# piljoong-jeong/nerf_meets_mlx

Measured on AMD Instinct MI355X. Metric: train+render rays/sec on Lego 800x800 (synthetic), coarse+fine 64+128, higher is better.
Workload: dtype split16 (fp16x2 render / bf16x2 train MFMA operands ~ 22 / 16 significand bits; fp32 accumulate)

## Files before the change

include/nerf_hip.h:

```cpp
#ifndef NERF_HIP_H
#define NERF_HIP_H

#include <stddef.h>
#include <stdint.h>

#ifdef __cplusplus
extern "C" {
#endif

#define NERF_ABI_VERSION 3

#define NERF_OK 0
#define NERF_E_NULL (-1)
#define NERF_E_SHAPE (-2)
#define NERF_E_UNSUPPORTED (-3)
#define NERF_E_HIP (-4)
#define NERF_E_RCCL (-5)

int nerf_abi_version(void);
const char* nerf_last_error(void);

#define NERF_RAY_STRIDE 11

int nerf_pixel_permutation(int64_t* out_idx, int64_t n, int64_t domain, uint64_t seed, uint64_t offset,
                           void* stream);

int nerf_ray_gen(const int64_t* pixel_idx, int64_t n, int H, int W, const double* K_host, const float* c2w_host,
                 float near, float far, float* rays, int64_t* coords, void* stream);

int nerf_sample_batch(int64_t n, int H, int W, uint64_t seed, uint64_t offset, const double* K_host, const float* c2w_host,
                      float near, float far, const float* image, float* rays, float* target, int64_t* pixel_idx,
                      void* stream);

int nerf_sample_batch_rgba(int64_t n, int H, int W, uint64_t seed, uint64_t offset, const double* K_host, const float* c2w_host,
                           float near, float far, const float* image, float* rays, float* target, int64_t* pixel_idx,
                           void* stream);

int nerf_gather_rows(const float* src, int64_t n_src, const int64_t* idx, int64_t n, int channels, float* out,
                     void* stream);

int nerf_ndc_rays(float* rays, int64_t n, int H, int W, float focal, float near, void* stream);

int nerf_sample_coarse(const float* rays, int64_t B, int n, int lindisp, float perturb, const float* t_rand,
                       float* z, void* stream);

int nerf_add_noise_z(const float* z_in, const float* t_rand, int64_t B, int n, float strength, float* z_out,
                     void* stream);

int nerf_importance_sample(const float* z, const float* weights, const float* u, int64_t B, int n, int N, float eps,
                           float* z_new, float* z_merged, float* cdf, int64_t* inds, void* stream);

int nerf_encode_freq(const float* x, int64_t M, int D, int n_freqs, int freq_mode, float* out, void* stream);

int nerf_encode_sinusoidal(const float* x, int64_t M, int D, int n_freqs, const float* freqs_host,
                           int include_input, float* out, void* stream);

int nerf_sh_encode(const float* dirs, int64_t M, int degree, float* out, void* stream);

int nerf_hashgrid_forward(const float* x, int64_t M, const float* tables, int L, int log2_T, int F,
                          const int* resolutions_host, float* out, void* stream);
int nerf_hashgrid_backward(const float* x, int64_t M, const float* d_out, int L, int log2_T, int F,
                           const int* resolutions_host, float* d_tables, void* stream);

int nerf_ngp_encode(const float* rays, const float* z, int64_t B, int n, const float* tables, int L, int log2_T,
                    int F, const int* resolutions_host, int sh_degree, float pos_scale, float pos_offset, float* x_out,
                    float* pts_out, void* stream);
int nerf_hashgrid_backward_rays(const float* rays, const float* z, int64_t B, int n, const float* d_out, int L,
                                int log2_T, int F, const int* resolutions_host, float pos_scale, float pos_offset,
                                float* d_tables, void* stream);

int nerf_hashgrid_backward_ex(const float* x, int64_t M, const float* d_out, int L, int log2_T, int F,
                              const int* resolutions_host, int level_lo, int level_hi, int fixed_point, void* d_tables,
                              void* stream);
int nerf_hashgrid_backward_rays_ex(const float* rays, const float* z, int64_t B, int n, const float* d_out, int L,
                                   int log2_T, int F, const int* resolutions_host, float pos_scale, float pos_offset,
                                   int level_lo, int level_hi, int fixed_point, void* d_tables, void* stream);

int nerf_hashgrid_forward_lw(const float* x, int64_t M, const float* tables, int L, int log2_T, int F,
                             const int* resolutions_host, const float* level_weights_host, float* out, void* stream);
int nerf_ngp_encode_lw(const float* rays, const float* z, int64_t B, int n, const float* tables, int L, int log2_T,
                       int F, const int* resolutions_host, const float* level_weights_host, int sh_degree,
                       float pos_scale, float pos_offset, float* x_out, float* pts_out, void* stream);
int nerf_hashgrid_backward_ex_lw(const float* x, int64_t M, const float* d_out, int L, int log2_T, int F,
                                 const int* resolutions_host, const float* level_weights_host, int level_lo,
                                 int level_hi, int fixed_point, void* d_tables, void* stream);
int nerf_hashgrid_backward_rays_ex_lw(const float* rays, const float* z, int64_t B, int n, const float* d_out, int L,
                                      int log2_T, int F, const int* resolutions_host, const float* level_weights_host,
                                      float pos_scale, float pos_offset, int level_lo, int level_hi, int fixed_point,
                                      void* d_tables, void* stream);

int nerf_composite_forward(const float* raw, const float* z, const float* rays, int64_t B, int n,
                           float raw_noise_std, const float* noise, int white_bkgd, float* rgb, float* disp,
                           float* acc, float* weights, float* depth, void* stream);

int nerf_composite_backward(const float* raw, const float* z, const float* rays, int64_t B, int n,
                            float raw_noise_std, const float* noise, int white_bkgd, const float* d_rgb,
                            const float* d_acc, const float* d_depth, float* d_raw, void* stream);

int nerf_mse_loss_grad(const float* pred, const float* target, int64_t count, float grad_scale, float* loss_out,
                       float* d_pred, void* stream);

int nerf_composite_mse_backward(const float* raw, const float* z, const float* rays, int64_t B, int n, int white_bkgd,
                                const float* target, float grad_scale, float* loss_out, float* rgb, float* d_raw,
                                void* stream);

int nerf_ssim_sums(const float* pred, const float* gt, int N, int C, int H, int W, const float* window_host,
                   int w_size, float c1, float c2, double* sums, void* stream);

typedef struct nerf_mlp_arch {
  int n_layers;
  int width;
  int in_pos;
  int in_dir;
  int skip_layer;
  int use_viewdirs;
  int out_ch;
  int precision;
} nerf_mlp_arch;

int64_t nerf_mlp_param_count(const nerf_mlp_arch* arch);
int64_t nerf_mlp_packed_bytes(const nerf_mlp_arch* arch);
int nerf_mlp_pack(const nerf_mlp_arch* arch, const float* params, void* packed, void* stream);

int64_t nerf_mlp_acts_bytes(const nerf_mlp_arch* arch, int64_t M);
int64_t nerf_mlp_dz_bytes(const nerf_mlp_arch* arch, int64_t M);

int nerf_mlp_forward(const nerf_mlp_arch* arch, const void* packed, const float* x, int64_t M, float* out,
                     void* stream);
int nerf_mlp_forward_train(const nerf_mlp_arch* arch, const void* packed, const float* x, int64_t M, float* out,
                           void* acts, void* stream);

int nerf_query_fused(const nerf_mlp_arch* arch, const void* packed, const float* rays, const float* z, int64_t B,
                     int n, int freq_mode, float* raw, void* acts, void* stream);

int nerf_mlp_backward(const nerf_mlp_arch* arch, const void* packed, const void* acts, const float* d_raw,
                      int64_t M, void* dz, float* grads, void* stream);
int nerf_mlp_backward_inputs(const nerf_mlp_arch* arch, const void* packed, const void* acts, const float* d_raw,
                             int64_t M, void* dz, float* grads, float* d_x, void* stream);

int nerf_mlp_debug_width(const nerf_mlp_arch* arch, int kind, int layer);
int nerf_mlp_debug_read(const nerf_mlp_arch* arch, const void* store, int kind, int layer, int64_t M, float* out,
                        void* stream);

int nerf_ngp_query_fused(const nerf_mlp_arch* arch, const void* packed, const float* rays, const float* z, int64_t B,
                         int n, const float* tables, int L, int log2_T, int F, const int* resolutions_host,
                         int sh_degree, float pos_scale, float pos_offset, float* raw, void* acts, void* stream);
int nerf_ngp_query_fused_h(const nerf_mlp_arch* arch, const void* packed, const float* rays, const float* z, int64_t B,
                           int n, const float* tables, const void* tables_half, int L, int log2_T, int F,
                           const int* resolutions_host, int sh_degree, float pos_scale, float pos_offset, float* raw,
                           void* acts, void* stream);
int nerf_ngp_query_fused_lw(const nerf_mlp_arch* arch, const void* packed, const float* rays, const float* z, int64_t B,
                            int n, const float* tables, const void* tables_half, int L, int log2_T, int F,
                            const int* resolutions_host, const float* level_weights_host, int sh_degree, float pos_scale,
                            float pos_offset, float* raw, void* acts, void* stream);


int nerf_occ_points(int log2_res, int64_t cell0, int64_t count, uint64_t seed, uint64_t update, float pos_scale,
                    float pos_offset, float* rays_out, float* z_out, void* stream);
int nerf_occ_merge(float* density, const float* raw, int64_t count, float decay, void* stream);
int64_t nerf_occ_finalize_workspace_bytes(int log2_res);
int nerf_occ_finalize(const float* density, int log2_res, float thr_cap, void* workspace, float* thr_out, uint32_t* bits,
                      void* stream);
int64_t nerf_occ_cull_workspace_bytes(int64_t B, int n);
int nerf_occ_cull(const float* rays, const float* z, int64_t B, int n, const uint32_t* bits, int log2_res, float pos_scale,
                  float pos_offset, void* workspace, int64_t* idx_out, int64_t* count_out, float* rays_out, float* z_out,
                  float* raw_fill, void* stream);
int nerf_scatter_rows(const float* src, const int64_t* idx, int64_t n, int channels, float* dst, int64_t n_dst, void* stream);

#define NERF_MARCH_MAX_STEPS 1024
int64_t nerf_occ_march_workspace_bytes(int64_t B);
int nerf_occ_march_count(const float* rays, int64_t B, const float* jitter, float jitter_const, const uint32_t* bits, int log2_res,
                         float pos_scale, float pos_offset, float step_world, int march_steps, void* workspace, int64_t* offsets,
                         void* stream);
int nerf_occ_march_write(const float* rays, int64_t B, const float* jitter, float jitter_const, const uint32_t* bits, int log2_res,
                         float pos_scale, float pos_offset, float step_world, int march_steps, void* workspace, int64_t* offsets,
                         float* rows_out, float* z_out, void* stream);
#define NERF_OCC_RELU 0
#define NERF_OCC_EXP 1
int nerf_occ_merge_ex(float* density, const float* raw, int64_t count, float decay, int activation, void* stream);

int nerf_composite_packed_forward(const float* raw, const float* z, const int64_t* offsets, int64_t B, int64_t K, float step_world,
                                  int white_bkgd, float* rgb, float* acc, float* depth, void* stream);
int nerf_composite_packed_mse_backward(const float* raw, const int64_t* offsets, int64_t B, int64_t K, float step_world,
                                       int white_bkgd, const float* target, float grad_scale, float* loss_out, float* rgb,
                                       float* d_raw, void* stream);

int nerf_composite_packed_distortion(const float* raw, const float* z, const int64_t* offsets, const float* rays, int64_t B,
                                     int64_t K, float step_world, int march_steps, int white_bkgd, float* rgb, float* acc,
                                     float* depth, float* dist, void* stream);
int nerf_composite_packed_mse_dist_backward(const float* raw, const float* z, const int64_t* offsets, const float* rays, int64_t B,
                                            int64_t K, float step_world, int march_steps, int white_bkgd, const float* target,
                                            float grad_scale, float dist_weight, float* loss_out, float* dist_out, float* rgb,
                                            float* d_raw, void* stream);

int nerf_composite_packed_forward_bg(const float* raw, const float* z, const int64_t* offsets, int64_t B, int64_t K, float step_world,
                                     const float* bg, int bg_stride, float* rgb, float* acc, float* depth, void* stream);
int nerf_composite_packed_distortion_bg(const float* raw, const float* z, const int64_t* offsets, const float* rays, int64_t B,
                                        int64_t K, float step_world, int march_steps, const float* bg, int bg_stride, float* rgb,
                                        float* acc, float* depth, float* dist, void* stream);
int nerf_composite_packed_mse_backward_bg(const float* raw, const int64_t* offsets, int64_t B, int64_t K, float step_world,
                                          const float* target_rgba, const float* bg, float grad_scale, float* loss_out, float* rgb,
                                          float* d_raw, void* stream);
int nerf_composite_packed_mse_dist_backward_bg(const float* raw, const float* z, const int64_t* offsets, const float* rays, int64_t B,
                                               int64_t K, float step_world, int march_steps, const float* target_rgba,
                                               const float* bg, float grad_scale, float dist_weight, float* loss_out,
                                               float* dist_out, float* rgb, float* d_raw, void* stream);

#define NERF_ERT_TERMINATED 1
int64_t nerf_ert_march_workspace_bytes(int64_t B);
int nerf_ert_init(int64_t B, int32_t* istate, float* fstate, int32_t* live, void* stream);
int nerf_ert_march_count(const float* rays, int64_t B, const float* jitter, float jitter_const, const uint32_t* bits, int log2_res,
                         float pos_scale, float pos_offset, float step_world, int march_steps, const int32_t* live, int64_t A,
                         const int32_t* istate, int max_new, void* workspace, int64_t* totals, void* stream);
int nerf_ert_march_write(const float* rays, int64_t B, const float* jitter, float jitter_const, const uint32_t* bits, int log2_res,
                         float pos_scale, float pos_offset, float step_world, int march_steps, const int32_t* live, int64_t A,
                         int32_t* istate, int max_new, void* workspace, int64_t* offsets, int32_t* live_out, float* rows_out,
                         float* z_out, void* stream);
int nerf_ert_fold(const float* raw, const float* z, const int64_t* offsets, const int32_t* live, int64_t A, int64_t B, int64_t K,
                  float step_world, float min_transmittance, int32_t* istate, float* fstate, void* stream);
int nerf_ert_finish(const int32_t* istate, const float* fstate, int64_t B, int white_bkgd, float* rgb, float* acc, float* depth,
                    int32_t* samples, void* stream);
int nerf_ert_finish_bg(const int32_t* istate, const float* fstate, int64_t B, const float* bg, int bg_stride, float* rgb, float* acc,
                       float* depth, int32_t* samples, void* stream);

#define NERF_MESH_MAX_RES 512
int64_t nerf_mesh_workspace_bytes(int res);
int nerf_mesh_points(int res, const float* lo_host, const float* hi_host, int64_t p0, int64_t count, float* rays_out, float* z_out,
                     void* stream);
int nerf_mesh_count(const float* vol, int res, float iso, void* workspace, int64_t* totals, void* stream);
int nerf_mesh_write_vertices(const float* vol, int res, float iso, const float* lo_host, const float* hi_host, void* workspace,
                             int64_t V, float* verts, float* normals, float* color_rows, void* stream);
int nerf_mesh_write_faces(const float* vol, int res, float iso, void* workspace, int64_t F, int32_t* faces, void* stream);

int64_t nerf_ccl_workspace_bytes(int res);
int nerf_ccl_label(const float* vol, int res, float iso, void* workspace, int32_t* labels, void* stream);
int nerf_ccl_sizes(const int32_t* labels, int res, int32_t* sizes, int64_t* stats, void* stream);
int nerf_ccl_filter(const float* vol, const int32_t* labels, const int32_t* sizes, const int64_t* stats, int res, float iso,
                    int64_t min_voxels, int largest_only, float* out, void* stream);

#define NERF_MORPH_MAX_RADIUS 16
int64_t nerf_morph_workspace_bytes(int res);
int nerf_morph_erode(const float* vol, int res, float iso, int radius, void* workspace, float* core, int64_t* stats2, void* stream);
int nerf_morph_reconstruct(const float* vol, const float* kept, int res, float iso, int radius, void* workspace, float* out,
                           int64_t* stats2, void* stream);


#define NERF_TSDF_MAX_VIEWS 16
typedef struct nerf_tsdf_view {
  float c2w[12];
  float fx, fy, cx, cy;
} nerf_tsdf_view;
int nerf_tsdf_reset(float* D, float* Wt, uint8_t* flags, int res, void* stream);
int nerf_tsdf_integrate(float* D, float* Wt, uint8_t* flags, int res, const float* lo_host, const float* hi_host,
                        const nerf_tsdf_view* views_host, int n, int H, int W, const float* depth, const float* acc, float trunc,
                        float acc_min, float far, int carve, void* stream);
int nerf_tsdf_volume(const float* D, const float* Wt, const uint8_t* flags, int res, int min_views, float* vol_out, void* stream);

#define NERF_SIMPLIFY_MEAN 0
#define NERF_SIMPLIFY_QUADRIC 1
int64_t nerf_simplify_workspace_bytes(int64_t V, int64_t F, int grid);
int nerf_simplify_cluster(const float* verts, const float* normals, const float* colors, int64_t V, const int32_t* faces, int64_t F,
                          const float* lo_host, const float* hi_host, int grid, void* workspace, int64_t* tri_keys, void* stream);
int nerf_simplify_count(const int64_t* sorted_keys, const int64_t* perm, int64_t V, const int32_t* faces, int64_t F, int grid,
                        void* workspace, int64_t* totals, void* stream);
int nerf_simplify_write(int64_t V, const int32_t* faces, int64_t F, const float* lo_host, const float* hi_host, int grid,
                        int placement, void* workspace, int64_t V_out, int64_t F_out, float* verts_out, float* normals_out,
                        float* colors_out, float* color_rows, int32_t* faces_out, void* stream);

int64_t nerf_smooth_workspace_bytes(int64_t V, int64_t F);
int nerf_smooth_build(int64_t V, const int32_t* faces, int64_t F, void* workspace, void* stream);
int nerf_smooth_run(const float* verts_in, int64_t V, const float* lo_host, const float* hi_host, int iterations, float lambda,
                    float mu, void* workspace, float* verts_out, void* stream);
int nerf_smooth_normals(const float* verts, int64_t V, const float* lo_host, const float* hi_host, void* workspace,
                        float* normals_out, float* color_rows, void* stream);

// ... 93 lines not shown
```

nerf_meets_mlx_amd/_native.py:

```python
import ctypes as C
import os

import torch

_HERE = os.path.dirname(os.path.abspath(__file__))
LIB_PATH = os.environ.get("NERF_HIP_LIB", os.path.join(_HERE, "libnerf_hip.so"))

_P, _I64, _I, _F, _U64 = C.c_void_p, C.c_int64, C.c_int, C.c_float, C.c_uint64
SIGNATURES = {
    "nerf_abi_version": (_I, []),
    "nerf_last_error": (C.c_char_p, []),
    "nerf_pixel_permutation": (_I, [_P, _I64, _I64, _U64, _U64, _P]),
    "nerf_ray_gen": (_I, [_P, _I64, _I, _I, C.POINTER(C.c_double), C.POINTER(C.c_float), _F, _F, _P, _P, _P]),
    "nerf_sample_batch": (_I, [_I64, _I, _I, _U64, _U64, C.POINTER(C.c_double), C.POINTER(C.c_float), _F, _F, _P, _P, _P, _P, _P]),
    "nerf_sample_batch_rgba": (_I, [_I64, _I, _I, _U64, _U64, C.POINTER(C.c_double), C.POINTER(C.c_float), _F, _F, _P, _P, _P, _P, _P]),
    "nerf_gather_rows": (_I, [_P, _I64, _P, _I64, _I, _P, _P]),
    "nerf_ndc_rays": (_I, [_P, _I64, _I, _I, _F, _F, _P]),
    "nerf_sample_coarse": (_I, [_P, _I64, _I, _I, _F, _P, _P, _P]),
    "nerf_add_noise_z": (_I, [_P, _P, _I64, _I, _F, _P, _P]),
    "nerf_importance_sample": (_I, [_P, _P, _P, _I64, _I, _I, _F, _P, _P, _P, _P, _P]),
    "nerf_encode_freq": (_I, [_P, _I64, _I, _I, _I, _P, _P]),
    "nerf_encode_sinusoidal": (_I, [_P, _I64, _I, _I, C.POINTER(C.c_float), _I, _P, _P]),
    "nerf_sh_encode": (_I, [_P, _I64, _I, _P, _P]),
    "nerf_hashgrid_forward": (_I, [_P, _I64, _P, _I, _I, _I, C.POINTER(C.c_int), _P, _P]),
    "nerf_hashgrid_backward": (_I, [_P, _I64, _P, _I, _I, _I, C.POINTER(C.c_int), _P, _P]),
    "nerf_ngp_encode": (_I, [_P, _P, _I64, _I, _P, _I, _I, _I, C.POINTER(C.c_int), _I, C.c_float, C.c_float, _P, _P, _P]),
    "nerf_ngp_query_fused": (_I, [_P, _P, _P, _P, _I64, _I, _P, _I, _I, _I, C.POINTER(C.c_int), _I, C.c_float, C.c_float, _P, _P, _P]),
    "nerf_ngp_query_fused_h": (_I, [_P, _P, _P, _P, _I64, _I, _P, _P, _I, _I, _I, C.POINTER(C.c_int), _I, C.c_float, C.c_float, _P, _P, _P]),
    "nerf_hashgrid_backward_rays": (_I, [_P, _P, _I64, _I, _P, _I, _I, _I, C.POINTER(C.c_int), C.c_float, C.c_float, _P, _P]),
    "nerf_hashgrid_backward_ex": (_I, [_P, _I64, _P, _I, _I, _I, C.POINTER(C.c_int), _I, _I, _I, _P, _P]),
    "nerf_hashgrid_backward_rays_ex": (_I, [_P, _P, _I64, _I, _P, _I, _I, _I, C.POINTER(C.c_int), C.c_float, C.c_float, _I, _I, _I, _P, _P]),
    "nerf_hashgrid_forward_lw": (_I, [_P, _I64, _P, _I, _I, _I, C.POINTER(C.c_int), C.POINTER(C.c_float), _P, _P]),
    "nerf_ngp_encode_lw": (_I, [_P, _P, _I64, _I, _P, _I, _I, _I, C.POINTER(C.c_int), C.POINTER(C.c_float), _I, C.c_float, C.c_float, _P, _P, _P]),
    "nerf_ngp_query_fused_lw": (_I, [_P, _P, _P, _P, _I64, _I, _P, _P, _I, _I, _I, C.POINTER(C.c_int), C.POINTER(C.c_float), _I, C.c_float, C.c_float, _P, _P, _P]),
    "nerf_hashgrid_backward_ex_lw": (_I, [_P, _I64, _P, _I, _I, _I, C.POINTER(C.c_int), C.POINTER(C.c_float), _I, _I, _I, _P, _P]),
    "nerf_hashgrid_backward_rays_ex_lw": (_I, [_P, _P, _I64, _I, _P, _I, _I, _I, C.POINTER(C.c_int), C.POINTER(C.c_float), C.c_float, C.c_float, _I, _I, _I, _P, _P]),
    "nerf_composite_forward": (_I, [_P, _P, _P, _I64, _I, _F, _P, _I, _P, _P, _P, _P, _P, _P]),
    "nerf_composite_backward": (_I, [_P, _P, _P, _I64, _I, _F, _P, _I, _P, _P, _P, _P, _P]),
    "nerf_mse_loss_grad": (_I, [_P, _P, _I64, _F, _P, _P, _P]),
    "nerf_composite_mse_backward": (_I, [_P, _P, _P, _I64, _I, _I, _P, _F, _P, _P, _P, _P]),
    "nerf_ssim_sums": (_I, [_P, _P, _I, _I, _I, _I, C.POINTER(C.c_float), _I, _F, _F, _P, _P]),
    "nerf_mlp_param_count": (_I64, [_P]),
    "nerf_mlp_packed_bytes": (_I64, [_P]),
    "nerf_mlp_pack": (_I, [_P, _P, _P, _P]),
    "nerf_mlp_acts_bytes": (_I64, [_P, _I64]),
    "nerf_mlp_dz_bytes": (_I64, [_P, _I64]),
    "nerf_mlp_forward": (_I, [_P, _P, _P, _I64, _P, _P]),
    "nerf_mlp_forward_train": (_I, [_P, _P, _P, _I64, _P, _P, _P]),
    "nerf_query_fused": (_I, [_P, _P, _P, _P, _I64, _I, _I, _P, _P, _P]),
    "nerf_mlp_backward": (_I, [_P, _P, _P, _P, _I64, _P, _P, _P]),
    "nerf_mlp_backward_inputs": (_I, [_P, _P, _P, _P, _I64, _P, _P, _P, _P]),
    "nerf_mlp_debug_width": (_I, [_P, _I, _I]),
    "nerf_mlp_debug_read": (_I, [_P, _P, _I, _I, _I64, _P, _P]),
    "nerf_render_workspace_bytes": (_I64, [_I64, _I, _I]),
    "nerf_render_rays_fused": (_I, [_P, _P, _P, _P, _I64, _I, _I, _P, _I, _I, _P, _P, _P, _P, _P, _P, _P, _P, _P, _P]),
    "nerf_comm_unique_id": (_I, [C.c_char_p]),
    "nerf_comm_init": (_I, [C.POINTER(C.c_void_p), _I, _I, C.c_char_p]),
    "nerf_allreduce_grads": (_I, [_P, _P, _I64, _P]),
    "nerf_comm_destroy": (_I, [_P]),
    "nerf_set_option": (_I, [C.c_char_p, _I]),
    "nerf_get_option": (_I, [C.c_char_p]),
    "nerf_adam_step": (_I, [_P, _P, _P, _P, _I64, _F, _F, _F, _F, _I, _I, _F, _P]),
    "nerf_adam_step_ex": (_I, [_P, _P, _P, _P, _I64, _F, _F, _F, _F, _I, _I, _F, _I, _I, _P]),
    "nerf_adam_step_shadow": (_I, [_P, _P, _P, _P, _I64, _F, _F, _F, _F, _I, _I, _F, _I, _I, _P, _P]),
    "nerf_occ_points": (_I, [_I, _I64, _I64, _U64, _U64, _F, _F, _P, _P, _P]),
    "nerf_occ_merge": (_I, [_P, _P, _I64, _F, _P]),
    "nerf_occ_finalize_workspace_bytes": (_I64, [_I]),
    "nerf_occ_finalize": (_I, [_P, _I, _F, _P, _P, _P, _P]),
    "nerf_occ_cull_workspace_bytes": (_I64, [_I64, _I]),
    "nerf_occ_cull": (_I, [_P, _P, _I64, _I, _P, _I, _F, _F, _P, _P, _P, _P, _P, _P, _P]),
    "nerf_scatter_rows": (_I, [_P, _P, _I64, _I, _P, _I64, _P]),
    "nerf_occ_merge_ex": (_I, [_P, _P, _I64, _F, _I, _P]),
    "nerf_occ_march_workspace_bytes": (_I64, [_I64]),
    "nerf_occ_march_count": (_I, [_P, _I64, _P, _F, _P, _I, _F, _F, _F, _I, _P, _P, _P]),
    "nerf_occ_march_write": (_I, [_P, _I64, _P, _F, _P, _I, _F, _F, _F, _I, _P, _P, _P, _P, _P]),
    "nerf_composite_packed_forward": (_I, [_P, _P, _P, _I64, _I64, _F, _I, _P, _P, _P, _P]),
    "nerf_composite_packed_mse_backward": (_I, [_P, _P, _I64, _I64, _F, _I, _P, _F, _P, _P, _P, _P]),
    "nerf_composite_packed_distortion": (_I, [_P, _P, _P, _P, _I64, _I64, _F, _I, _I, _P, _P, _P, _P, _P]),
    "nerf_composite_packed_mse_dist_backward": (_I, [_P, _P, _P, _P, _I64, _I64, _F, _I, _I, _P, _F, _F, _P, _P, _P, _P, _P]),
    "nerf_composite_packed_forward_bg": (_I, [_P, _P, _P, _I64, _I64, _F, _P, _I, _P, _P, _P, _P]),
    "nerf_composite_packed_distortion_bg": (_I, [_P, _P, _P, _P, _I64, _I64, _F, _I, _P, _I, _P, _P, _P, _P, _P]),
    "nerf_composite_packed_mse_backward_bg": (_I, [_P, _P, _I64, _I64, _F, _P, _P, _F, _P, _P, _P, _P]),
    "nerf_composite_packed_mse_dist_backward_bg": (_I, [_P, _P, _P, _P, _I64, _I64, _F, _I, _P, _P, _F, _F, _P, _P, _P, _P, _P]),
    "nerf_ert_march_workspace_bytes": (_I64, [_I64]),
    "nerf_ert_init": (_I, [_I64, _P, _P, _P, _P]),
    "nerf_ert_march_count": (_I, [_P, _I64, _P, _F, _P, _I, _F, _F, _F, _I, _P, _I64, _P, _I, _P, _P, _P]),
    "nerf_ert_march_write": (_I, [_P, _I64, _P, _F, _P, _I, _F, _F, _F, _I, _P, _I64, _P, _I, _P, _P, _P, _P, _P, _P]),
    "nerf_ert_fold": (_I, [_P, _P, _P, _P, _I64, _I64, _I64, _F, _F, _P, _P, _P]),
    "nerf_ert_finish": (_I, [_P, _P, _I64, _I, _P, _P, _P, _P, _P]),
    "nerf_ert_finish_bg": (_I, [_P, _P, _I64, _P, _I, _P, _P, _P, _P, _P]),
    "nerf_mesh_workspace_bytes": (_I64, [_I]),
    "nerf_mesh_points": (_I, [_I, C.POINTER(C.c_float), C.POINTER(C.c_float), _I64, _I64, _P, _P, _P]),
    "nerf_mesh_count": (_I, [_P, _I, _F, _P, _P, _P]),
    "nerf_mesh_write_vertices": (_I, [_P, _I, _F, C.POINTER(C.c_float), C.POINTER(C.c_float), _P, _I64, _P, _P, _P, _P]),
    "nerf_mesh_write_faces": (_I, [_P, _I, _F, _P, _I64, _P, _P]),
    "nerf_ccl_workspace_bytes": (_I64, [_I]),
    "nerf_ccl_label": (_I, [_P, _I, _F, _P, _P, _P]),
    "nerf_ccl_sizes": (_I, [_P, _I, _P, _P, _P]),
    "nerf_ccl_filter": (_I, [_P, _P, _P, _P, _I, _F, _I64, _I, _P, _P]),
    "nerf_morph_workspace_bytes": (_I64, [_I]),
    "nerf_morph_erode": (_I, [_P, _I, _F, _I, _P, _P, _P, _P]),
    "nerf_morph_reconstruct": (_I, [_P, _P, _I, _F, _I, _P, _P, _P, _P]),
    "nerf_tsdf_reset": (_I, [_P, _P, _P, _I, _P]),
    "nerf_tsdf_integrate": (_I, [_P, _P, _P, _I, C.POINTER(C.c_float), C.POINTER(C.c_float), C.POINTER(C.c_float), _I, _I, _I, _P, _P,
                                _F, _F, _F, _I, _P]),
    "nerf_tsdf_volume": (_I, [_P, _P, _P, _I, _I, _P, _P]),
    "nerf_simplify_workspace_bytes": (_I64, [_I64, _I64, _I]),
    "nerf_simplify_cluster": (_I, [_P, _P, _P, _I64, _P, _I64, C.POINTER(C.c_float), C.POINTER(C.c_float), _I, _P, _P, _P]),
    "nerf_simplify_count": (_I, [_P, _P, _I64, _P, _I64, _I, _P, _P, _P]),
    "nerf_simplify_write": (_I, [_I64, _P, _I64, C.POINTER(C.c_float), C.POINTER(C.c_float), _I, _I, _P, _I64, _I64, _P, _P, _P, _P,
                                _P, _P]),
    "nerf_smooth_workspace_bytes": (_I64, [_I64, _I64]),
    "nerf_smooth_build": (_I, [_I64, _P, _I64, _P, _P]),
    "nerf_smooth_run": (_I, [_P, _I64, C.POINTER(C.c_float), C.POINTER(C.c_float), _I, _F, _F, _P, _P, _P]),
    "nerf_smooth_normals": (_I, [_P, _I64, C.POINTER(C.c_float), C.POINTER(C.c_float), _P, _P, _P, _P]),
    "nerf_texture_layout": (_I, [_I64, _I, C.POINTER(C.c_int64)]),
    "nerf_texture_rows": (_I, [_P, _P, _I64, _P, _I64, _I, _I64, _I64, _P, _P]),
    "nerf_texture_store": (_I, [_P, _I64, _P, _I64, _I, _I64, _I64, _P, _P]),
    "nerf_texture_uv": (_I, [_I64, _I, _P, _P]),
    "nerf_texture_sample": (_I, [_P, _P, _P, _I64, _P, _I64, _I, _P, _P, _I64, _P, _P, _P]),
    "nerf_raster_clear": (_I, [_P, _I, _I, _P, _P]),
    "nerf_raster_draw": (_I, [_P, _I64, _P, _I64, _I64, C.POINTER(C.c_float), _I, _I, _F, _I, _I, _P, _P, _P]),
    "nerf_raster_resolve": (_I, [_P, _P, _I64, _P, _I64, C.POINTER(C.c_float), _I, _I, _F, _P, _P, _P, _P, _P]),
    "nerf_raster_shade": (_I, [_P, _P, _P, _I64, _I64, _P, _P, _P, _I, _I, _I, _P, _P]),
    "nerf_project_accumulate": (_I, [_P, _P, _I64, _P, _I64, _I, _I64, _I64, C.POINTER(C.c_float), _I, _I, _I, _P, _P, _P, _F, _F, _F, _F,
                                    _I, _P, _P]),
    "nerf_project_finish": (_I, [_P, _I64, _I, _I64, _I64, _I, _P, _P, _P, _P]),
    "nerf_mip_levels": (_I, [_I, C.POINTER(C.c_int32)]),
    "nerf_mip_reduce": (_I, [_P, _I64, _I, _P, _I64, _I64, _P]),
    "nerf_mip_lod": (_I, [_P, _I64, _P, _I64, C.POINTER(C.c_float), _F, _I, _F, _P, _P]),
    "nerf_mip_sample": (_I, [C.POINTER(C.c_void_p), _I64, _I, _P, _P, _P, _I, _I64, _P, _P]),
    "nerf_surface_cdf_workspace_bytes": (_I64, [_I64]),
    "nerf_surface_cdf": (_I, [_P, _I64, _P, _I64, C.POINTER(C.c_float), C.POINTER(C.c_float), _P, _P, _P]),
    "nerf_surface_sample": (_I, [_P, _I64, _P, _I64, _P, _I64, _I64, _U64, _P, _P, _P]),
    "nerf_meshdist_workspace_bytes": (_I64, [_I64, _I]),
    "nerf_meshdist_count": (_I, [_P, _I64, _P, _I64, C.POINTER(C.c_float), C.POINTER(C.c_float), _I, _P, _P, _P]),
    "nerf_meshdist_build": (_I, [_P, _I64, _P, _I64, C.POINTER(C.c_float), C.POINTER(C.c_float), _I, _P, _P, _I64, _P]),
    "nerf_meshdist_query": (_I, [_P, _I64, _P, _I64, _P, _I64, C.POINTER(C.c_float), C.POINTER(C.c_float), _I, _P, _P, _I64, _P, _P,
                                _P]),
    "nerf_bvh_workspace_bytes": (_I64, [_I64]),
    "nerf_bvh_keys": (_I, [_P, _I64, _P, _I64, C.POINTER(C.c_float), C.POINTER(C.c_float), _P, _P]),
    "nerf_bvh_build": (_I, [_P, _I64, _P, _I64, _P, _P, _P]),
    "nerf_bvh_query": (_I, [_P, _I64, _P, _I64, _P, _I64, C.POINTER(C.c_float), C.POINTER(C.c_float), _P, _P, _P, _P]),
    "nerf_closest_points": (_I, [_P, _I64, _P, _I64, _P, _I64, _P, _P, _P]),
}


class MlpArch(C.Structure):
    _fields_ = [("n_layers", _I), ("width", _I), ("in_pos", _I), ("in_dir", _I), ("skip_layer", _I),
                ("use_viewdirs", _I), ("out_ch", _I), ("precision", _I)]


class NerfHipError(RuntimeError):
    pass


_lib = None


def lib():
    global _lib
    if _lib is None:
        if not os.path.exists(LIB_PATH):
            raise NerfHipError(
                f"{LIB_PATH} not found: build it with `python -c 'import __graft_entry__ as g; g.build()'` "
                "(hipcc --offload-arch=gfx950).  There is no CPU fallback.")
        L = C.CDLL(LIB_PATH)
        for name, (res, args) in SIGNATURES.items():
            fn = getattr(L, name)
            fn.restype, fn.argtypes = res, args
        _lib = L
    return _lib


def check(rc: int):
    if rc != 0:
        msg = lib().nerf_last_error().decode(errors="replace")
        if rc in (-1, -2, -3):
            raise ValueError(f"libnerf_hip error {rc}: {msg}")
        raise NerfHipError(f"libnerf_hip error {rc}: {msg}")


def ptr(t):
    if t is None:
        return None
    if not t.is_cuda:
        raise ValueError("libnerf_hip kernels need tensors on the ROCm device (there is no CPU path)")
    if not t.is_contiguous():
        raise ValueError("libnerf_hip kernels need contiguous tensors")
    return C.c_void_p(t.data_ptr())


def stream():
    return C.c_void_p(torch.cuda.current_stream().cuda_stream)


def f32(t, device=None):
    if not torch.is_tensor(t):
        t = torch.as_tensor(t)
    if device is not None:
        t = t.to(device)
    return t.to(torch.float32).contiguous()
```

nerf_meets_mlx_amd/csrc/mlp.hip:

```cpp
#include "common.h"
#include "mlp_ring.h"
#include "mlp_layout.h"
#include "mlp_frag.h"
#include "mlp_arch2.h"
#include "mlp_input2.h"
#include "mlp_pack.h"
#include "hash_common.h"
#include "mlp_params.h"
#include "mlp_model.h"
#include "dw_split.h"
#include <limits.h>
#include <string.h>


namespace nerf {

extern int g_hash_combine_max_res;








template <int ST, int KS, int NT, bool RELU, bool MASKOUT, class WS, class SINK = NoSink>
__device__ __forceinline__ void layer_fwd(WS& ws, int fbase, int bias_slot, const bf16x8 (&in)[ST][KS],
                                          bf16x8 (&out)[ST][2 * NT], u32x4 (&mask)[ST], int lane,
                                          const SINK& sink = SINK()) {
  const int h = lane >> 5;
  f32x16 prev[ST];
#pragma unroll
  for (int nt = 0; nt < NT; ++nt) {
    f32x16 acc[ST];
    acc_init_bias(acc[0], ws, bias_slot + 32 * nt, h);
#pragma unroll
    for (int t = 1; t < ST; ++t) acc[t] = acc[0];
#pragma unroll
    for (int ks = 0; ks < KS; ++ks) {
      const bf16x8 a = next_frag(ws, fbase + nt * KS + ks, lane);
#pragma unroll
      for (int t = 0; t < ST; ++t) acc[t] = __builtin_amdgcn_mfma_f32_32x32x16_bf16(a, in[t][ks], acc[t], 0, 0, 0);
      if (nt > 0) {
#pragma unroll
        for (int q = 0; q < 4; ++q)
          if (quarter_pos(KS, q) == ks) {
#pragma unroll
            for (int t = 0; t < ST; ++t) {
              finish_quarter<RELU, MASKOUT>(prev[t], q, nt - 1, out[t][2 * nt - 2], out[t][2 * nt - 1], mask[t]);
              if (q == 3) { sink.put(t, 2 * nt - 2, out[t][2 * nt - 2]); sink.put(t, 2 * nt - 1, out[t][2 * nt - 1]); }
            }
          }
      }
    }
#pragma unroll
    for (int t = 0; t < ST; ++t) prev[t] = acc[t];
  }
#pragma unroll
  for (int q = 0; q < 4; ++q)
#pragma unroll
    for (int t = 0; t < ST; ++t)
      finish_quarter<RELU, MASKOUT>(prev[t], q, NT - 1, out[t][2 * NT - 2], out[t][2 * NT - 1], mask[t]);
#pragma unroll
  for (int t = 0; t < ST; ++t) { sink.put(t, 2 * NT - 2, out[t][2 * NT - 2]); sink.put(t, 2 * NT - 1, out[t][2 * NT - 1]); }
}


template <int ST, int MODE, bool STORE, class WS>
__device__ __forceinline__ void fwd_tiles(const FwdArgs& a, WS& ws, int64_t tile0, int64_t ntiles, int lane, PassQueue* pq = nullptr) {
  const int r = lane & 31, h = lane >> 5;
  bf16x8 pe[ST][4], dpe[ST][2];
  if (pq) pq->ask(ws_wave(ws), lane);
#pragma unroll
  for (int t = 0; t < ST; ++t) {
    int64_t tile = tile0 + t; if (tile >= ntiles) tile = ntiles - 1;
    const int64_t m = clamp_sample(tile * 32 + r, a.M);
    if (MODE == 0) {
      const float* row = a.x + m * 90;
#pragma unroll
      for (int ks = 0; ks < 4; ++ks) row_pairs<CvtBf16>(row, ks, h, 63, pe[t][ks]);
#pragma unroll
      for (int ks = 0; ks < 2; ++ks) row_pairs<CvtBf16>(row + 63, ks, h, 27, dpe[t][ks]);
    } else {
      const Sample sm = load_sample(a.rays, a.z, m, a.n);
#if NERF_ABLATE == 3
      for (int q = 0; q < 4; ++q) for (int j = 0; j < 8; ++j) pe[t][q][j] = (__bf16)sm.p[j % 3];
      for (int q = 0; q < 2; ++q) for (int j = 0; j < 8; ++j) dpe[t][q][j] = (__bf16)sm.d[j % 3];
      if (false)
#endif
      {
      encode_pairs<SinRevFract, CvtBf16, 0, 63, 10>(sm.p, a.fr.pos, h, pe[t][0]); encode_pairs<SinRevFract, CvtBf16, 1, 63, 10>(sm.p, a.fr.pos, h, pe[t][1]);
      encode_pairs<SinRevFract, CvtBf16, 2, 63, 10>(sm.p, a.fr.pos, h, pe[t][2]); encode_pairs<SinRevFract, CvtBf16, 3, 63, 10>(sm.p, a.fr.pos, h, pe[t][3]);
      encode_pairs<SinRevFract, CvtBf16, 0, 27, 4>(sm.d, a.fr.dir, h, dpe[t][0]); encode_pairs<SinRevFract, CvtBf16, 1, 27, 4>(sm.d, a.fr.dir, h, dpe[t][1]);
      }
    }
  }
  if (pq) pq->publish(ws_wave(ws));
  int bad[ST];
#pragma unroll
  for (int t = 0; t < ST; ++t)
  {
    bad[t] = nonfinite_flags<32>(nonfinite_bits(pe[t][0]) | nonfinite_bits(pe[t][1]) | nonfinite_bits(pe[t][2]) | nonfinite_bits(pe[t][3]),
                                 nonfinite_bits(dpe[t][0]) | nonfinite_bits(dpe[t][1]));
    asm volatile("" : "+v"(bad[t]));
  }
#define store(slot0, t, frags, count) \
  do { if (STORE) { store_frags<count>(a.acts, tile0 + (t), a.astride, slot0, frags, r, h); ws.note_stores(count); } } while (0)
#pragma unroll
  for (int t = 0; t < ST; ++t) { store(L::A_PE, t, pe[t], 4); store(L::A_DPE, t, dpe[t], 2); }

  bf16x8 ha[ST][16], hb[ST][16];
  u32x4 mk[ST];
#define SINK(slot0) FragSink<STORE>{a.acts, tile0, a.astride, slot0, r, h}
#define MASK_BEGIN() do { _Pragma("unroll") for (int t = 0; t < ST; ++t) mk[t] = u32x4{0u, 0u, 0u, 0u}; } while (0)
#define MASK_STORE(layer) do { if (STORE) { _Pragma("unroll") for (int t = 0; t < ST; ++t) \
    *reinterpret_cast<u32x4*>(frag_ptr(a.acts, tile0 + t, a.astride, L::A_MASK + (layer), r, h)) = mk[t]; ws.note_stores(ST); } } while (0)
  MASK_BEGIN();
  layer_fwd<ST, 4, 8, true, STORE>(ws, L::F_L0, 0, pe, ha, mk, lane, SINK(L::A_H0));
  MASK_STORE(0);
  MASK_BEGIN();
  layer_fwd<ST, 16, 8, true, STORE>(ws, L::F_L1 + 0 * 128, 256, ha, hb, mk, lane, SINK(L::A_H0 + 16));
  MASK_STORE(1);
  MASK_BEGIN();
  layer_fwd<ST, 16, 8, true, STORE>(ws, L::F_L1 + 1 * 128, 512, hb, ha, mk, lane, SINK(L::A_H0 + 32));
  MASK_STORE(2);
  MASK_BEGIN();
  layer_fwd<ST, 16, 8, true, STORE>(ws, L::F_L1 + 2 * 128, 768, ha, hb, mk, lane, SINK(L::A_H0 + 48));
  MASK_STORE(3);
  MASK_BEGIN();
  layer_fwd<ST, 16, 8, true, STORE>(ws, L::F_L1 + 3 * 128, 1024, hb, ha, mk, lane, SINK(L::A_H0 + 64));
  MASK_STORE(4);
  {
    bf16x8 cat[ST][20];
#pragma unroll
    for (int t = 0; t < ST; ++t) {
      if (STORE && is_ring<WS>::value) {
#pragma unroll
        for (int k = 0; k < 4; ++k) pe[t][k] = *frag_ptr(a.acts, tile0 + t, a.astride, L::A_PE + k, r, h);
      }
#pragma unroll
      for (int k = 0; k < 4; ++k) cat[t][k] = pe[t][k];
#pragma unroll
      for (int k = 0; k < 16; ++k) cat[t][4 + k] = ha[t][k];
    }
    MASK_BEGIN();
    layer_fwd<ST, 20, 8, true, STORE>(ws, L::F_L5, 1280, cat, hb, mk, lane, SINK(L::A_H0 + 80));
    MASK_STORE(5);
  }
  MASK_BEGIN();
  layer_fwd<ST, 16, 8, true, STORE>(ws, L::F_L6, 1536, hb, ha, mk, lane, SINK(L::A_H0 + 96));
  MASK_STORE(6);
  MASK_BEGIN();
  layer_fwd<ST, 16, 8, true, STORE>(ws, L::F_L7, 1792, ha, hb, mk, lane, SINK(L::A_H0 + 112));
  MASK_STORE(7);
  layer_fwd<ST, 16, 8, false, false>(ws, L::F_FA, L::BI_FEAT, hb, ha, mk, lane, SINK(L::A_FEAT));
  float alpha[ST];
  {
    f32x16 acc[ST];
    acc_init_bias(acc[0], ws, L::BI_ALPHA, h);
#pragma unroll
    for (int t = 1; t < ST; ++t) acc[t] = acc[0];
#pragma unroll
    for (int ks = 0; ks < 16; ++ks) {
      const bf16x8 wa = next_frag(ws, L::F_FA + 128 + ks, lane);
#pragma unroll
      for (int t = 0; t < ST; ++t) acc[t] = __builtin_amdgcn_mfma_f32_32x32x16_bf16(wa, hb[t][ks], acc[t], 0, 0, 0);
    }
#pragma unroll
    for (int t = 0; t < ST; ++t) alpha[t] = acc[t][0];
  }
// ... 786 lines not shown
  }
  ws.drain();
}



struct LdsW {
  __device__ __forceinline__ bf16x8 frag(int f, int lane) { return *reinterpret_cast<const bf16x8*>(ring_smem + f * 1024 + lane * 16); }
  __device__ __forceinline__ void note_stores(int) {}
  __device__ __forceinline__ float4 bias4(int slot) { return *reinterpret_cast<const float4*>(ring_smem + 32 * 1024 + slot * 4); }
};
__device__ __forceinline__ void lds_load_stream(const bf16x8* __restrict__ w, const float* __restrict__ bias) {
  for (int i = threadIdx.x; i < 32 * 64; i += blockDim.x) *reinterpret_cast<bf16x8*>(ring_smem + i * 16) = w[i];
  if (bias)
    for (int i = threadIdx.x; i < LN::BI_TOTAL; i += blockDim.x) *reinterpret_cast<float*>(ring_smem + 32 * 1024 + 4 * i) = bias[i];
  __syncthreads();
}


template <bool STORE, bool FUSED, bool LW = false>
__global__ void __launch_bounds__(512) mlp_small_fwd_kernel(SmallArgs a) {
  constexpr int ST = 1;
  lds_load_stream(a.wf, a.bias);
  const int lane0 = threadIdx.x & 63, wv = threadIdx.x >> 6;
  const bool rmaj = FUSED && !STORE && a.ray_major;
  const int64_t ntiles = rmaj ? ((a.B + 31) >> 5) * a.n : (a.M + 31) >> 5;
  LdsW ws;
  for (int64_t tile0 = (int64_t)blockIdx.x * 8 + wv; tile0 < ntiles; tile0 += (int64_t)gridDim.x * 8) {
    int lane = lane0;
    asm volatile("" : "+v"(lane));
    const int r = lane & 31, h = lane >> 5;
    const TileSample ts = small_tile_sample(a, tile0, r, rmaj);
    const int64_t m = ts.m;
    const bool valid = ts.valid;
    bf16x8 in[3];
    if (FUSED) {
      if (a.tables_h) ngp_row<true, LW, CvtBf16>(a, m, h, in);
      else ngp_row<false, LW, CvtBf16>(a, m, h, in);
    } else {
      small_row<CvtBf16>(a.x + m * LN::CIN, h, in);
    }
    bf16x8 xin[ST][2], din[ST][1];
    xin[0][0] = in[0]; xin[0][1] = in[1]; din[0][0] = in[2];
    int bad = nonfinite_flags<32>(nonfinite_bits(xin[0][0]) | nonfinite_bits(xin[0][1]), nonfinite_bits(din[0][0]));
    asm volatile("" : "+v"(bad));
#define SINK(slot0) FragSink<STORE>{a.acts, tile0, a.astride, slot0, r, h}
#define MASK_STORE(layer) do { if (STORE) *reinterpret_cast<u32x4*>(frag_ptr(a.acts, tile0, a.astride, LN::A_MASK + (layer), r, h)) = mk[0]; } while (0)
    if (STORE) { store_frags<2>(a.acts, tile0, a.astride, LN::A_X, xin[0], r, h); store_frags<1>(a.acts, tile0, a.astride, LN::A_DX, din[0], r, h); }
    u32x4 mk[ST];
    bf16x8 h0[ST][4], h1[ST][4], ft[ST][4];
    mk[0] = u32x4{0u, 0u, 0u, 0u};
    layer_fwd<ST, 2, 2, true, STORE>(ws, LN::F_L0, LN::BI_L0, xin, h0, mk, lane, SINK(LN::A_H0));
    MASK_STORE(0);
    mk[0] = u32x4{0u, 0u, 0u, 0u};
    layer_fwd<ST, 4, 2, true, STORE>(ws, LN::F_L1, LN::BI_L1, h0, h1, mk, lane, SINK(LN::A_H1));
    MASK_STORE(1);
    layer_fwd<ST, 4, 2, false, false>(ws, LN::F_FA, LN::BI_FEAT, h1, ft, mk, lane, SINK(LN::A_FEAT));
    float alpha;
    {
      f32x16 acc;
      acc_init_bias(acc, ws, LN::BI_ALPHA, h);
#pragma unroll
      for (int ks = 0; ks < 4; ++ks) acc = __builtin_amdgcn_mfma_f32_32x32x16_bf16(ws.frag(LN::F_FA + 8 + ks, lane), h1[0][ks], acc, 0, 0, 0);
      alpha = acc[0];
    }
    bf16x8 hd[ST][2];
    {
      bf16x8 cat[ST][5];
#pragma unroll
      for (int k = 0; k < 4; ++k) cat[0][k] = ft[0][k];
      cat[0][4] = din[0][0];
      mk[0] = u32x4{0u, 0u, 0u, 0u};
      layer_fwd<ST, 5, 1, true, STORE>(ws, LN::F_DIR, LN::BI_DIR, cat, hd, mk, lane, SINK(LN::A_HD));
      MASK_STORE(2);
    }
    {
      f32x16 acc;
      acc_init_bias(acc, ws, LN::BI_RGB, h);
#pragma unroll
      for (int ks = 0; ks < 2; ++ks) acc = __builtin_amdgcn_mfma_f32_32x32x16_bf16(ws.frag(LN::F_RGB + ks, lane), hd[0][ks], acc, 0, 0, 0);
      if (h == 0 && valid) {
        float4 o; o.x = acc[0]; o.y = acc[1]; o.z = acc[2]; o.w = alpha;
        *reinterpret_cast<float4*>(a.out + m * 4) = poison_raw(o, bad);
      }
    }
#undef SINK
#undef MASK_STORE
  }
}

__global__ void __launch_bounds__(512) mlp_small_bwd_kernel(SmallArgs a) {
  constexpr int ST = 1;
  lds_load_stream(a.wb, nullptr);
  const int lane0 = threadIdx.x & 63, wv = threadIdx.x >> 6;
  const int64_t ntiles = (a.M + 31) >> 5;
  LdsW ws;
  for (int64_t tile0 = (int64_t)blockIdx.x * 8 + wv; tile0 < ntiles; tile0 += (int64_t)gridDim.x * 8) {
    int lane = lane0;
    asm volatile("" : "+v"(lane));
    const int r = lane & 31, h = lane >> 5;
    const int64_t m = tile0 * 32 + r;
    float4 g = make_float4(0.f, 0.f, 0.f, 0.f);
    if (m < a.M && h == 0) g = *reinterpret_cast<const float4*>(a.d_raw + m * 4);
    bf16x8 zrgb[ST][1], zal[ST][1];
#pragma unroll
    for (int j = 0; j < 8; ++j) { zrgb[0][0][j] = (__bf16)0.0f; zal[0][0][j] = (__bf16)0.0f; }
    zrgb[0][0][0] = (__bf16)g.x; zrgb[0][0][1] = (__bf16)g.y; zrgb[0][0][2] = (__bf16)g.z;
    zal[0][0][0] = (__bf16)g.w;
    u32x4 mk[3][ST];
#pragma unroll
    for (int l = 0; l < 3; ++l)
      mk[l][0] = *reinterpret_cast<const u32x4*>(frag_ptr(const_cast<void*>(a.acts), tile0, a.astride, LN::A_MASK + l, r, h));
    store_frags<1>(a.dz, tile0, a.zstride, LN::Z_RGB, zrgb[0], r, h);
    store_frags<1>(a.dz, tile0, a.zstride, LN::Z_A, zal[0], r, h);
#define ZSINK(slot0) FragSink<true>{a.dz, tile0, a.zstride, slot0, r, h}
    bf16x8 zd[ST][2], zf[ST][4], z1[ST][4], z0[ST][4];
    layer_bwd<ST, 1, 1, true>(ws, LN::B_RGB, zrgb, zd, mk[2], lane, ZSINK(LN::Z_D));
    layer_bwd<ST, 2, 2, false>(ws, LN::B_DIR, zd, zf, mk[2], lane, ZSINK(LN::Z_F));
    {
      bf16x8 cat[ST][5];
#pragma unroll
      for (int k = 0; k < 4; ++k) cat[0][k] = zf[0][k];
      cat[0][4] = zal[0][0];
      layer_bwd<ST, 5, 2, true>(ws, LN::B_FA, cat, z1, mk[1], lane, ZSINK(LN::Z_L1));
    }
    layer_bwd<ST, 4, 2, true>(ws, LN::B_L1, z1, z0, mk[0], lane, ZSINK(LN::Z_L0));
#undef ZSINK
    if (a.d_x) {
      f32x16 acc;
#pragma unroll
      for (int i = 0; i < 16; ++i) acc[i] = 0.0f;
#pragma unroll
      for (int ns = 0; ns < 4; ++ns) acc = __builtin_amdgcn_mfma_f32_32x32x16_bf16(ws.frag(LN::B_L0 + ns, lane), z0[0][ns], acc, 0, 0, 0);
      if (m < a.M) {
#pragma unroll
        for (int q = 0; q < 4; ++q) {
          float4 o; o.x = acc[4 * q]; o.y = acc[4 * q + 1]; o.z = acc[4 * q + 2]; o.w = acc[4 * q + 3];
          *reinterpret_cast<float4*>(a.d_x + m * LN::CPOS + 8 * q + 4 * h) = o;
        }
      }
    }
  }
}

static int g_dw_wgs = 0;
static int g_dw_bias = -1;
static int g_bwd_stage = 0;
static int g_dw_ring_cap = 8;
static int g_dw_private = 4;
static int g_dw16_variant = 1;
static int g_dw_narrow_first = 1;
static int g_dw_factor = 1;
static int g_train_fold = 0;
static int g_dw_job_mask = 0;
static int g_mlp_variant = 0;
static int g_ring_wgs = 0;
static int g_ngp_ray_major = 1;
int g_pass_queue = 1;
static int g_ring_split = 1;

static int cu_count() {
  constexpr int MAX_DEVICES = 64;
  static int n[MAX_DEVICES] = {};
  int dev = 0;
  if (hipGetDevice(&dev) != hipSuccess || dev < 0 || dev >= MAX_DEVICES) dev = 0;
  if (n[dev] == 0) {
    int v = 0;
    n[dev] = (hipDeviceGetAttribute(&v, hipDeviceAttributeMultiprocessorCount, dev) == hipSuccess && v > 0) ? v : 256;
  }
  return n[dev];
}
static inline bool dw_factored(const Model& m) { return g_dw_factor && m.can_factor() && !g_dw_job_mask && s16::g_dw_variant != 0; }
static inline bool train_folded(const Model& m) { return g_train_fold && dw_factored(m); }
static inline int ring_wgs() { return g_ring_wgs > 0 ? g_ring_wgs : cu_count(); }
static inline unsigned ring_grid(int64_t ntiles) { return persistent_grid((ntiles + 7) / 8, ring_wgs()); }

struct Option { const char* key; int* var; bool (*rule)(int& v); const char* refusal; };
static bool opt_any(int&) { return true; }
static bool opt_flag(int& v) { v = v ? 1 : 0; return true; }
template <int LO, int HI> static bool opt_clamp(int& v) { v = v < LO ? LO : v > HI ? HI : v; return true; }
static const Option OPTIONS[] = {
    {"mlp_variant", &g_mlp_variant, opt_any, nullptr},
    {"ring_split", &g_ring_split, [](int& v) { return v == 1 || v == 2; }, "nerf_set_option: ring_split must be 1 or 2"},
    {"ring_workgroups", &g_ring_wgs, opt_clamp<0, INT_MAX>, nullptr},
    {"tile_pad16", &g_tile_pad16, opt_clamp<0, INT_MAX>, nullptr},
    {"dw_workgroups", &g_dw_wgs, opt_clamp<0, INT_MAX>, nullptr},
    {"dw_unit_bias", &g_dw_bias, opt_clamp<-1, INT_MAX>, nullptr},
    {"bwd_stage", &g_bwd_stage, opt_any, nullptr},
    {"dw_job_mask", &g_dw_job_mask, opt_any, nullptr},
    {"hash_combine_max_res", &g_hash_combine_max_res, opt_clamp<0, INT_MAX>, nullptr},
    {"ngp_ray_major", &g_ngp_ray_major, opt_flag, nullptr},
    {"dw22_variant", &s16::g_dw_variant, opt_flag, nullptr},
    {"dw16_variant", &g_dw16_variant, opt_clamp<0, 3>, nullptr},
    {"dw_private_tiles", &g_dw_private, opt_clamp<0, 4>, nullptr},
    {"dw_ring_cap", &g_dw_ring_cap, opt_clamp<2, 16>, nullptr},
    {"pass_queue", &g_pass_queue, opt_flag, nullptr},
    {"dw_narrow_first", &g_dw_narrow_first, opt_flag, nullptr},
    {"dw_factor", &g_dw_factor, opt_flag, nullptr},
    {"train_fold", &g_train_fold, opt_flag, nullptr},
    {"f22_tiles", &f22::g_tiles, [](int& v) { return v == 0 || v == 2 || v == 3; }, "nerf_set_option: f22_tiles must be 0 (automatic), 2 or 3"},
};

}

using namespace nerf;

extern "C" int nerf_set_option(const char* key, int value) {
  NERF_REQUIRE(key, NERF_E_NULL, "nerf_set_option: key is NULL");
  NERF_REQUIRE(strcmp(key, "mlp_precision") != 0, NERF_E_UNSUPPORTED,
               "nerf_set_option: \"mlp_precision\" is gone (ABI 3): set nerf_mlp_arch.precision of the model instead");
  for (const Option& o : OPTIONS) {
    if (strcmp(key, o.key)) continue;
    if (!o.rule(value)) return fail(NERF_E_UNSUPPORTED, "%s", o.refusal);
    *o.var = value;
    return NERF_OK;
  }
  return fail(NERF_E_UNSUPPORTED, "nerf_set_option: unknown key '%s'", key);
}

extern "C" int nerf_get_option(const char* key) {
  if (!key) return NERF_OPTION_UNKNOWN;
  for (const Option& o : OPTIONS)
    if (!strcmp(key, o.key)) return *o.var;
  return NERF_OPTION_UNKNOWN;
}

extern "C" int64_t nerf_mlp_param_count(const nerf_mlp_arch* arch) { return resolve(arch).params; }
extern "C" int64_t nerf_mlp_packed_bytes(const nerf_mlp_arch* arch) { return resolve(arch).packed_bytes; }
extern "C" int64_t nerf_mlp_acts_bytes(const nerf_mlp_arch* arch, int64_t M) { return resolve(arch).acts_bytes(M); }
extern "C" int64_t nerf_mlp_dz_bytes(const nerf_mlp_arch* arch, int64_t M) { return resolve(arch).dz_bytes(M); }

#define NERF_ARCH_MSG ": HIP kernels exist for (8x256, skip 4) with in=63+27 view head, or in=40 / no view head / out_ch<=4, and for (2x64, no skip) with in=32+16 view head"
#define NERF_RESOLVE(who)        \
  const Model m = resolve(arch); \
  NERF_REQUIRE(m.ok, NERF_E_UNSUPPORTED, who NERF_ARCH_MSG)

extern "C" int nerf_mlp_pack(const nerf_mlp_arch* arch, const float* params, void* packed, void* stream) {
  NERF_RESOLVE("nerf_mlp_pack");
  NERF_REQUIRE(params && packed, NERF_E_NULL, "nerf_mlp_pack: params/packed is NULL");
  auto s = as_stream(stream);
  bf16x8* wf = m.stream<bf16x8>(packed, S_FWD);
  bf16x8* wb = m.stream<bf16x8>(packed, S_BWD);
  float* bias = m.stream<float>(packed, S_BIAS);
  int rc;
  if (m.shape == Shape::Small) {
    rc = launch<pack_streams_kernel<SmallPack, CvtBf16, true>>("nerf_mlp_pack (2x64 model)", dim3(pack_blocks<SmallPack, true>()), dim3(256), 0, s,
                                                               params, wf, wb, bias, 0);
    if (!rc && m.split()) rc = s16x::small_pack(params, m.stream<void>(packed, S_S16), s);
  } else if (m.shape == Shape::Image) {
    rc = launch<pack_streams_kernel<ImgPack, CvtBf16, true>>("nerf_mlp_pack (image model)", dim3(pack_blocks<ImgPack, true>()), dim3(256), 0, s,
                                                             params, wf, wb, bias, m.out_ch);
    if (!rc && m.split()) rc = s16x::img_pack(params, m.out_ch, m.stream<void>(packed, S_S16), s);
    if (!rc && m.prec == Prec::F32) rc = f32::pack(params, m.stream<void>(packed, S_F32), m.out_ch, s);
  } else {
    rc = launch<pack_kernel>("nerf_mlp_pack", dim3(PACK_BLOCKS + PACK16_BLOCKS), dim3(256), 0, s, params, wf, wb, bias,
                             m.stream<bf16x8>(packed, S_FWD16));
    if (!rc && m.prec == Prec::F32) rc = f32::pack(params, m.stream<void>(packed, S_F32), 0, s);
    if (!rc && m.split()) rc = f22::pack(params, m.stream<void>(packed, S_F22), s);
    if (!rc && m.split()) rc = s16::pack(params, m.stream<void>(packed, S_S16), train_folded(m), s);
  }
  return rc;
}

template <int MODE>
static int launch_fwd(const Model& m, const void* packed, const float* x, const float* rays, const float* z, int64_t M, int n,
                      int freq_mode, float* out, void* acts, void* stream) {
  FwdArgs a;
  a.queue = nullptr;
  a.wf = m.stream<bf16x8>(packed, S_FWD);
  a.bias = m.stream<float>(packed, S_BIAS);
  a.x = x; a.rays = rays; a.z = z; a.M = M; a.n = n; a.out = out; a.acts = acts; a.astride = m.astride();
  fill_freqs(a.fr.pos, a.fr.dir, freq_mode);
  const int64_t ntiles = (M + 31) / 32;
  auto s = as_stream(stream);
  const int variant = (g_mlp_variant == 0) ? (MODE == 1 ? (acts ? 3 : 4) : 1) : g_mlp_variant;
  if ((variant == 4 || variant == 5) && MODE == 1 && !acts) {
    const dim3 g(persistent_grid((M + 255) / 256, ring_wgs()));
    FwdArgs a16 = a;
    a16.queue = passq_slot();
    a16.wf = m.stream<bf16x8>(packed, S_FWD16);
    const char* what = "mlp forward (ring, 16x16x32)";
    if (variant == 4) return launch<mlp_fwd_ring16_kernel<8, 2>, mlp_fwd_ring16_kernel<4, 4>>(what, g, dim3(512), RING16_LDS_BYTES, s, a16);
    return launch<mlp_fwd_ring16_kernel<4, 4>, mlp_fwd_ring16_kernel<8, 2>>(what, g, dim3(256), RING16_LDS_BYTES, s, a16);
  }
  if (variant >= 3 && MODE == 1) {
    a.queue = passq_slot();
    if (acts && g_ring_split == 2) {
      return launch<mlp_fwd_ring_kernel<1, true, SPLIT_NW, SPLIT_CHUNK>>(
          "mlp forward (ring, 2 workgroups per CU)", dim3(persistent_grid((ntiles + SPLIT_NW - 1) / SPLIT_NW, 2 * (int64_t)ring_wgs())),
          dim3(64 * SPLIT_NW), SPLIT_LDS_BYTES, s, a);
    }
    return with_bool(acts != nullptr, [&](auto store) {
      constexpr bool ST = decltype(store)::value;
      return launch<mlp_fwd_ring_kernel<1, ST>, mlp_fwd_ring_kernel<1, !ST>>("mlp forward (ring)", dim3(ring_grid(ntiles)), dim3(512),
                                                                              RING_LDS_BYTES, s, a);
    });
  }
  const int st = variant == 2 ? 2 : 1;
  const int64_t blocks = (ntiles + 4 * st - 1) / (4 * st);
  NERF_REQUIRE(blocks < (1ll << 31), NERF_E_SHAPE, "mlp forward: M too large");
  return with_bool(st == 1, [&](auto one) { return with_bool(acts != nullptr, [&](auto store) {
    return launch<mlp_fwd_kernel<decltype(one)::value ? 1 : 2, MODE, decltype(store)::value>>("mlp forward", dim3((unsigned)blocks), dim3(256),
                                                                                                0, s, a);
  }); });
}


static int view_forward(const Model& m, const void* packed, const float* x, const float* rays, const float* z, int64_t M, int n,
                        int freq_mode, float* out, void* acts, void* stream);

extern "C" int nerf_mlp_forward_train(const nerf_mlp_arch* arch, const void* packed, const float* x, int64_t M,
                                      float* out, void* acts, void* stream) {
  NERF_RESOLVE("nerf_mlp_forward");
  if (M <= 0) return NERF_OK;
  NERF_REQUIRE(packed && x && out, NERF_E_NULL, "nerf_mlp_forward: NULL pointer");
  auto s = as_stream(stream);
  if (m.shape == Shape::Small) {
    SmallArgs a;
    small_args(a, m, packed);
    a.x = x; a.out = out; a.acts = acts; a.M = M;
    if (m.split()) return s16x::small_forward(a, false, dim3(small_grid(small_tiles(a))), s);
    return with_bool(acts != nullptr, [&](auto store) {
      return launch<mlp_small_fwd_kernel<decltype(store)::value, false>>("mlp forward (2x64 model)", dim3(small_grid((M + 31) / 32)), dim3(512),
                                                                         LN::LDS_BYTES, s, a);
    });
  }
  if (m.shape == Shape::Image) {
    if (m.prec == Prec::F32)
      return f32::forward(m.stream<void>(packed, S_F32), x, nullptr, nullptr, M, 1, 0, out, acts, m.out_ch, s);
    ImgArgs a;
    img_args(a, m, packed);
    a.x = x; a.out = out; a.acts = acts; a.M = M;
    if (m.split()) return s16x::img_forward(a, ring_wgs(), s);
    return with_bool(acts != nullptr, [&](auto store) {
      constexpr bool ST = decltype(store)::value;
      return launch<mlp_img_fwd_ring_kernel<ST>, mlp_img_fwd_ring_kernel<!ST>>("mlp forward (image model)", dim3(ring_grid((M + 31) / 32)),
                                                                               dim3(512), RING_LDS_BYTES, s, a);
    });
  }
  return view_forward(m, packed, x, nullptr, nullptr, M, 1, 0, out, acts, stream);
}

static int view_forward(const Model& m, const void* packed, const float* x, const float* rays, const float* z, int64_t M, int n,
                        int freq_mode, float* out, void* acts, void* stream) {
  auto s = as_stream(stream);
  if (m.split() && !acts)
    return f22::forward(m.stream<void>(packed, S_F22), x, rays, z, M, n, freq_mode, out, ring_wgs(), s);
  if (m.split())
    return s16::forward(m.stream<void>(packed, S_S16), m.stream<float>(packed, S_BIAS), x, rays, z, M, n, freq_mode, out, acts,
                        m.astride(), ring_wgs(), train_folded(m), s);
  if (m.prec == Prec::F32) return f32::forward(m.stream<void>(packed, S_F32), x, rays, z, M, n, freq_mode, out, acts, 0, s);
  return x ? launch_fwd<0>(m, packed, x, rays, z, M, n, freq_mode, out, acts, stream)
           : launch_fwd<1>(m, packed, x, rays, z, M, n, freq_mode, out, acts, stream);
}

extern "C" int nerf_mlp_forward(const nerf_mlp_arch* arch, const void* packed, const float* x, int64_t M, float* out,
                                void* stream) {
  return nerf_mlp_forward_train(arch, packed, x, M, out, nullptr, stream);
}

extern "C" int nerf_query_fused(const nerf_mlp_arch* arch, const void* packed, const float* rays, const float* z,
                                int64_t B, int n, int freq_mode, float* raw, void* acts, void* stream) {
  const Model m = resolve(arch);
  NERF_REQUIRE(m.ok && m.shape == Shape::View, NERF_E_UNSUPPORTED, "nerf_query_fused" NERF_ARCH_MSG);
  NERF_REQUIRE(n >= 1, NERF_E_SHAPE, "nerf_query_fused: n must be >= 1");
  if (B <= 0) return NERF_OK;
  NERF_REQUIRE(packed && rays && z && raw, NERF_E_NULL, "nerf_query_fused: NULL pointer");
  NERF_REQUIRE(freq_mode == 0 || freq_mode == 1, NERF_E_UNSUPPORTED, "nerf_query_fused: freq_mode must be 0 or 1");
  NERF_REQUIRE(B * (int64_t)n < (1ll << 31), NERF_E_SHAPE, "nerf_query_fused: B*n must be < 2^31 samples per call");
  return view_forward(m, packed, nullptr, rays, z, B * n, n, freq_mode, raw, acts, stream);
}

static int launch_dw_part(const Model& m, DwArgs& d, int nj, int64_t ntiles, const void* acts, void* dz, float* grads,
                          hipStream_t s, int kind, int slot_base, int max_wgs, int aux_slot = -1) {
  static_assert(DW_SPLIT_MAX_JOBS == DW_MAX_JOBS, "dw_split.h sizes its arrays for DwArgs::jobs");
  DwCost cost[DW_MAX_JOBS];
  constexpr int SHARED_JOB_EXTRA_UNITS = 12;
  for (int j = 0; j < nj; ++j) cost[j] = DwCost{d.jobs[j].nf, d.jobs[j].kf + (d.jobs[j].aux_row0 > 0 ? SHARED_JOB_EXTRA_UNITS : 0)};
  int target_wgs = g_dw_wgs > 0 ? g_dw_wgs : cu_count();
  if (target_wgs > max_wgs) target_wgs = max_wgs;
  const int nw = dw_split(cost, nj, g_dw_bias >= 0 ? g_dw_bias : m.split() ? 2 : 128, target_wgs, (ntiles + 3) / 4, d.splits);
  NERF_REQUIRE(slot_base + nw <= DW_MAX_WGS, NERF_E_SHAPE, "nerf_mlp_backward: dw_workgroups must be <= %d", DW_MAX_WGS);
  bool all_tiny = true;
  for (int j = 0; j < nj; ++j) all_tiny = all_tiny && ((d.jobs[j].nf + 1) / 2) * ((d.jobs[j].kf + 1) / 2) <= 4;
  d.ntiles = (int)ntiles; d.astride = m.astride(); d.zstride = m.zstride();
  d.acts = acts; d.dz = dz; d.grads = grads;
  d.a_lo = m.info->a_lo; d.z_lo = m.info->z_lo; d.ring_cap = g_dw_ring_cap; d.private_max_tiles = g_dw_private;
  d.partial = m.dw_partial(dz, ntiles) + (size_t)slot_base * DW_SLOT_FLOATS;
  d.aux = aux_slot >= 0 ? m.dw_partial(dz, ntiles) + (size_t)aux_slot * DW_SLOT_FLOATS : nullptr;
  int rc;
  if (kind >= 2) {
    rc = launch_dw_wide_kernel(d, nw, kind == 2, s);
  } else if (kind == 1) {
    rc = s16::launch_dw_kernel(d, nw, true, s);
  } else if (g_dw16_variant == 3 || (g_dw16_variant == 1 && all_tiny)) {
    rc = s16::launch_dw_kernel(d, nw, false, s);
  } else {
    rc = launch<mlp_dw_kernel>("mlp dW", dim3(nw), dim3(64 * DW_WAVES), DW_LDS_BYTES, s, d);
  }
  if (rc) return rc;
  return launch<mlp_dw_reduce_kernel>("mlp dW reduce", dim3(257, nj), dim3(256), 0, s, d);
}

static int launch_dw(const Model& m, const void* packed, DwArgs& d, int nj, int64_t ntiles, const void* acts, void* dz, float* grads,
                     hipStream_t s, bool factored) {
  if (g_dw_job_mask) {
    hipError_t e = hipMemsetAsync(grads, 0, sizeof(float) * m.params, s);
    if (e != hipSuccess) return fail(NERF_E_HIP, "nerf_mlp_backward: memset: %s", hipGetErrorString(e));
  }
  const bool split_bf16 = m.split();
  if ((split_bf16 ? s16::g_dw_variant : g_dw16_variant) == 0)
    return launch_dw_part(m, d, nj, ntiles, acts, dz, grads, s, split_bf16 ? 1 : 0, 0, DW_MAX_WGS);
// ... 210 lines not shown
```

nerf_meets_mlx_amd/csrc/mlp22.h:

```cpp
#pragma once
#ifdef __HIPCC__
#include <hip/hip_runtime.h>
#endif
#include <stdint.h>
#include "mlp_index.h"

#ifndef NERF_F22_FOLD
#define NERF_F22_FOLD 1
#endif

namespace nerf {
namespace f22 {

constexpr int P_L0 = 0, P_L1 = 32, P_L5 = 544, P_L6 = 704, P_L7 = 832, P_HEADS = 960;
#if NERF_F22_FOLD
constexpr int P_ALPHA = P_HEADS, P_DIR = P_ALPHA + 8, P_RGB = P_DIR + 72, F_PAIRS = P_RGB + 4;
#else
constexpr int P_FEAT = P_HEADS, P_ALPHA = P_FEAT + 128, P_DIR = P_ALPHA + 8, P_RGB = P_DIR + 72, F_PAIRS = P_RGB + 4;
#endif
constexpr int F_CHUNK = 32;
constexpr int F_FRAGS = 2 * F_PAIRS, F_STREAM = (F_FRAGS + F_CHUNK - 1) / F_CHUNK * F_CHUNK, CHUNKS = F_STREAM / F_CHUNK;
constexpr int F_PADDED = 2368, BIAS_FLOATS = 2496;
constexpr int64_t PACKED_BYTES = (int64_t)F_PADDED * 1024 + (int64_t)BIAS_FLOATS * 4;
static_assert(F_STREAM <= F_PADDED && F_FRAGS % 4 == 0, "f22 stream layout");

#if NERF_F22_FOLD
constexpr int SRC_ZERO = -1, SRC_FOLD = -2;
struct Src { int p, n, k; };
__host__ __device__ constexpr Src src_param(int p) { return Src{p, 0, 0}; }
__host__ __device__ constexpr Src src_pos_chan(int row_base, int ks, int g, int j) {
  return pos_chan16(ks, g, j) >= 0 ? src_param(row_base + pos_chan16(ks, g, j)) : Src{SRC_ZERO, 0, 0};
}
__host__ __device__ constexpr Src stream_src(int fp, int i, int g, int j) {
  if (fp < P_L1) return src_pos_chan(L::P_W0 + (16 * (fp / 2) + i) * 63, fp % 2, g, j);
  if (fp < P_L5 || (fp >= P_L6 && fp < P_HEADS)) {
    const int q = fp < P_L5 ? fp - P_L1 : fp - P_L6, l = (fp < P_L5 ? 1 : 6) + q / 128, r = q % 128;
    return src_param(L::pw(l) + (16 * (r / 8) + i) * 256 + kperm16(r % 8, g, j));
  }
  if (fp < P_L6) {
    const int q = fp - P_L5, n = 16 * (q / 10) + i, ks = q % 10;
    return ks < 2 ? src_pos_chan(L::P_W5 + n * 319, ks, g, j) : src_param(L::P_W5 + n * 319 + 63 + kperm16(ks - 2, g, j));
  }
  if (fp < P_DIR) return i == 0 ? src_param(L::P_WA + kperm16(fp - P_ALPHA, g, j)) : Src{SRC_ZERO, 0, 0};
  if (fp < P_RGB) {
    const int q = fp - P_DIR, n = 16 * (q / 9) + i, ks = q % 9;
    if (ks < 8) return Src{SRC_FOLD, n, kperm16(ks, g, j)};
    return dir_chan16(g, j) >= 0 ? src_param(L::P_WD + n * 283 + 256 + dir_chan16(g, j)) : Src{SRC_ZERO, 0, 0};
  }
  if (fp < F_PAIRS) return i < 3 ? src_param(L::P_WR + i * 128 + kperm16(fp - P_RGB, g, j)) : Src{SRC_ZERO, 0, 0};
  return Src{SRC_ZERO, 0, 0};
}
#endif

#ifdef __HIPCC__
extern int g_tiles;
int pack(const float* params, void* packed22, hipStream_t s);
int forward(const void* packed22, const float* x, const float* rays, const float* z, int64_t M, int n, int freq_mode,
            float* out, int persistent_wgs, hipStream_t s);
#endif

}
}
```

nerf_meets_mlx_amd/csrc/mlp22.hip:

```cpp
#include "mlp_layout.h"
#include "mlp22.h"

#ifndef NERF_F22_PIN
#define NERF_F22_PIN 1
#endif
#ifndef NERF_F22_AGPR
#define NERF_F22_AGPR 1
#endif
#ifndef NERF_F22_MIXSUB
#define NERF_F22_MIXSUB 1
#endif
#ifndef NERF_F22_RG3
#define NERF_F22_RG3 4
#endif
#ifndef NERF_F22_PARK
#define NERF_F22_PARK (NERF_F22_FOLD ? 2 : 1)
#endif
#ifndef NERF_F22_IGLP
#define NERF_F22_IGLP 0
#endif

namespace nerf {
namespace f22 {

typedef _Float16 h8 __attribute__((ext_vector_type(8)));
typedef _Float16 h2 __attribute__((ext_vector_type(2)));
typedef float f32x2 __attribute__((ext_vector_type(2)));
typedef unsigned int u32x4 __attribute__((ext_vector_type(4)));

constexpr float LO_SCALE = 2048.0f, LO_INV = 1.0f / 2048.0f;
constexpr float F16_MIN_NORMAL = 6.103515625e-05f;
static_assert(F_CHUNK == RING_CHUNK && CHUNKS == (F_FRAGS + RING_CHUNK - 1) / RING_CHUNK && CHUNKS * RING_CHUNK <= F_PADDED, "f22 ring chunks");
static_assert(P_L0 == L16::F_L0 && P_L1 == L16::F_L1 && P_L5 == L16::F_L5 && P_L6 == L16::F_L6 && P_L7 == L16::F_L7 && P_HEADS == L16::F_FA, "f22 trunk");
#if NERF_F22_FOLD
static_assert(F_PAIRS == L::F16_TOTAL - 128 && CHUNKS == 66 && F_FRAGS % RING_CHUNK == (2 * L::F16_TOTAL) % RING_CHUNK, "f22 folded stream");
#else
static_assert(F_PAIRS == L::F16_TOTAL && P_ALPHA == L16::F_FA + 128 && P_DIR == L16::F_DIR && P_RGB == L16::F_RGB && CHUNKS == 74, "f22 stream layout");
#endif

struct HiLo { unsigned hi, lo; };
__device__ __forceinline__ HiLo split2(float v0, float v1) {
  const f32x2 v = {v0, v1};
  const h2 hh = __builtin_convertvector(v, h2);
#if NERF_F22_MIXSUB
  const f32x2 r = {__builtin_fmaf((float)hh[0], -LO_SCALE, v0 * LO_SCALE), __builtin_fmaf((float)hh[1], -LO_SCALE, v1 * LO_SCALE)};
#else
  const f32x2 r = {(v0 - (float)hh[0]) * LO_SCALE, (v1 - (float)hh[1]) * LO_SCALE};
#endif
  return HiLo{__builtin_bit_cast(unsigned, hh), __builtin_bit_cast(unsigned, __builtin_convertvector(r, h2))};
}

constexpr int PACK_THREADS = (F_PADDED / 2) * 64 + BIAS_FLOATS;
__global__ void __launch_bounds__(256) pack22_kernel(const float* __restrict__ p, u32x4* __restrict__ wf,
                                                     float* __restrict__ bias) {
  const int t = blockIdx.x * 256 + threadIdx.x;
  if (t < (F_PADDED / 2) * 64) {
    const int fp = t >> 6, lane = t & 63;
    u32x4 hi = {0u, 0u, 0u, 0u}, lo = {0u, 0u, 0u, 0u};
    if (fp < F_PAIRS) {
#if NERF_F22_FOLD
      float fold[8] = {0.0f, 0.0f, 0.0f, 0.0f, 0.0f, 0.0f, 0.0f, 0.0f};
      if (fp >= P_DIR && fp < P_RGB && (fp - P_DIR) % 9 < 8) {
        const float* __restrict__ wd = p + L::P_WD + (16 * ((fp - P_DIR) / 9) + (lane & 15)) * 283;
        const float* __restrict__ wfk = p + L::P_WF + kperm16((fp - P_DIR) % 9, lane >> 4, 0);
        double acc[8] = {0.0, 0.0, 0.0, 0.0, 0.0, 0.0, 0.0, 0.0};
#pragma unroll 4
        for (int f = 0; f < 256; ++f) {
          const double a = (double)wd[f];
#pragma unroll
          for (int e = 0; e < 8; ++e) acc[e] = __builtin_fma(a, (double)wfk[f * 256 + 16 * (e >> 2) + (e & 3)], acc[e]);
        }
#pragma unroll
        for (int e = 0; e < 8; ++e) fold[e] = (float)acc[e];
      }
#endif
#pragma unroll
      for (int j = 0; j < 8; j += 2) {
        float w[2];
        _Float16 wh[2], wl[2];
#pragma unroll
        for (int e = 0; e < 2; ++e) {
#if NERF_F22_FOLD
          const Src src = stream_src(fp, lane & 15, lane >> 4, j + e);
          w[e] = src.p >= 0 ? p[src.p] : src.p == SRC_FOLD ? fold[j + e] : 0.0f;
#else
          w[e] = fwd_src16(p, fp, lane & 15, lane >> 4, j + e);
#endif
          wh[e] = __builtin_fabsf(w[e]) < F16_MIN_NORMAL ? (_Float16)0.0f : (_Float16)w[e];
          wl[e] = (_Float16)((w[e] - (float)wh[e]) * LO_SCALE);
        }
        const h2 a = {wh[0], wh[1]}, b = {wl[0], wl[1]};
        hi[j >> 1] = __builtin_bit_cast(unsigned, a);
        lo[j >> 1] = __builtin_bit_cast(unsigned, b);
      }
    }
    wf[(2 * fp) * 64 + lane] = hi;
    wf[(2 * fp + 1) * 64 + lane] = lo;
  } else if (t < PACK_THREADS) {
    const int s = t - (F_PADDED / 2) * 64;
    float v = 0.0f;
    if (s < 2048) v = p[L::pb(s >> 8) + (s & 255)];
#if NERF_F22_FOLD
    else if (s < L::BI_ALPHA) v = 0.0f;
    else if (s < L::BI_DIR) v = (s == L::BI_ALPHA) ? p[L::P_BA] : 0.0f;
    else if (s < L::BI_RGB) {
      const float* __restrict__ wd = p + L::P_WD + (s - L::BI_DIR) * 283;
      double acc = 0.0;
      for (int f = 0; f < 256; ++f) acc = __builtin_fma((double)wd[f], (double)p[L::P_BF + f], acc);
      v = (float)(acc + (double)p[L::P_BD + (s - L::BI_DIR)]);
    }
#else
    else if (s < L::BI_ALPHA) v = p[L::P_BF + (s - L::BI_FEAT)];
    else if (s < L::BI_DIR) v = (s == L::BI_ALPHA) ? p[L::P_BA] : 0.0f;
    else if (s < L::BI_RGB) v = p[L::P_BD + (s - L::BI_DIR)];
#endif
    else v = (s - L::BI_RGB) < 3 ? p[L::P_BR + (s - L::BI_RGB)] : 0.0f;
    bias[s] = v;
  }
}

template <int COUNT>
__device__ __forceinline__ void split_slots(const float (&v)[COUNT], u32x4* hi, u32x4* lo) {
#pragma unroll
  for (int j = 0; j < COUNT; j += 2) {
    const HiLo q = split2(v[j], v[j + 1]);
    hi[j >> 3][(j & 7) >> 1] = q.hi; lo[j >> 3][(j & 7) >> 1] = q.lo;
  }
}
struct SplitF16 {
  static __device__ __forceinline__ void pack(const float (&v)[8], u32x4& hi, u32x4& lo) { split_slots<8>(v, &hi, &lo); }
};

__device__ __forceinline__ f32x4 mfma16(const u32x4& a, const u32x4& b, const f32x4& c) {
#if NERF_ABLATE == 41 || NERF_ABLATE == 42
  return c;
#endif
  return __builtin_amdgcn_mfma_f32_16x16x32_f16(__builtin_bit_cast(h8, a), __builtin_bit_cast(h8, b), c, 0, 0, 0);
}

template <int NS, int KS, int NT, bool RELU, class WS, int PARK_LDS = 0>
__device__ __forceinline__ void layer22(WS& ws, int pbase, int bias_slot, const u32x4 (&ih)[NS][KS], const u32x4 (&il)[NS][KS],
                                        u32x4 (&oh)[NS][NT / 2], u32x4 (&ol)[NS][NT / 2], int lane, unsigned park_addr = 0u, unsigned park2_addr = 0u) {
  const int g = lane >> 4;
  f32x4 pm[NS], pc[NS];
  if (PARK_LDS) asm volatile("ds_write_b128 %0, %1" :: "v"(park_addr), "v"(il[NS - 1][KS - 1]) : "memory");
  if (PARK_LDS >= 2)
    asm volatile("ds_write_b32 %0, %1\n\tds_write_b32 %0, %2 offset:1024\n\tds_write_b32 %0, %3 offset:2048\n\tds_write_b32 %0, %4 offset:6144"
                 :: "v"(park2_addr), "v"(il[NS - 2][KS - 1][0]), "v"(il[NS - 2][KS - 1][1]), "v"(il[NS - 2][KS - 1][2]), "v"(il[NS - 2][KS - 1][3]) : "memory");
#if NERF_F22_IGLP >= 0
  __builtin_amdgcn_iglp_opt(NERF_F22_IGLP);
#endif
  constexpr int NP = 2 * NS;
  auto piece = [&](int nt, int pcs, f32x4 (&m)[NS], f32x4 (&c)[NS]) {
    const int s = pcs >> 1, i = 2 * (pcs & 1);
#if NERF_ABLATE == 41 || NERF_ABLATE == 42
    return;
#endif
#if NERF_F22_PIN
    if (pcs == 0) {
#pragma unroll
      for (int t = 0; t < NS; ++t) asm volatile("" : "+v"(m[t]), "+v"(c[t]));
    }
#endif
    float v0 = __builtin_fmaf(c[s][i], LO_INV, m[s][i]), v1 = __builtin_fmaf(c[s][i + 1], LO_INV, m[s][i + 1]);
    if (RELU) { v0 = __builtin_elementwise_maximum(v0, 0.0f); v1 = __builtin_elementwise_maximum(v1, 0.0f); }
    const HiLo q = split2(v0, v1);
    oh[s][nt >> 1][2 * (nt & 1) + (i >> 1)] = q.hi; ol[s][nt >> 1][2 * (nt & 1) + (i >> 1)] = q.lo;
#if NERF_F22_AGPR
    if ((nt & 1) && i == 2) asm volatile("" : "+a"(oh[s][nt >> 1]), "+a"(ol[s][nt >> 1]));
#endif
  };
  auto piece_at = [](int q) { return NS == 2 ? (KS >= 8 ? 1 + 2 * q : (q * KS) / 4) : (KS >= 8 ? 1 + (q * (KS - 1)) / NP : (q * KS) / NP); };
#pragma unroll
  for (int nt = 0; nt < NT; ++nt) {
    const float4 b = ws.bias4(bias_slot + 16 * nt + 4 * g);
    f32x4 m[NS], c[NS];
    m[0][0] = b.x; m[0][1] = b.y; m[0][2] = b.z; m[0][3] = b.w;
    c[0] = f32x4{0.0f, 0.0f, 0.0f, 0.0f};
#pragma unroll
    for (int t = 1; t < NS; ++t) { m[t] = m[0]; c[t] = c[0]; }
#pragma unroll
    for (int ks = 0; ks < KS; ++ks) {
      const int fp = pbase + nt * KS + ks;
      const u32x4 ah = __builtin_bit_cast(u32x4, next_frag(ws, 2 * fp, lane));
      const u32x4 al = __builtin_bit_cast(u32x4, next_frag(ws, 2 * fp + 1, lane));
      if (NS == 2) {
        m[0] = mfma16(ah, ih[0][ks], m[0]);
        c[0] = mfma16(ah, il[0][ks], c[0]);
        m[1] = mfma16(ah, ih[1][ks], m[1]);
        c[1] = mfma16(ah, il[1][ks], c[1]);
        c[0] = mfma16(al, ih[0][ks], c[0]);
        c[1] = mfma16(al, ih[1][ks], c[1]);
      } else {
#pragma unroll
        for (int t = 0; t < NS; ++t) {
          m[t] = mfma16(ah, ih[t][ks], m[t]);
          if (PARK_LDS && t == NS - 1 && ks == KS - 1) {
            u32x4 b;
            asm volatile("ds_read_b128 %0, %1\n\ts_waitcnt lgkmcnt(0)" : "=v"(b) : "v"(park_addr) : "memory");
            c[t] = mfma16(ah, b, c[t]);
          } else if (PARK_LDS >= 2 && t == NS - 2 && ks == KS - 1) {
            u32x4 b;
            asm volatile("ds_read_b32 %0, %4\n\tds_read_b32 %1, %4 offset:1024\n\tds_read_b32 %2, %4 offset:2048\n\tds_read_b32 %3, %4 offset:6144\n\ts_waitcnt lgkmcnt(0)"
                         : "=&v"(b[0]), "=&v"(b[1]), "=&v"(b[2]), "=&v"(b[3]) : "v"(park2_addr) : "memory");
            c[t] = mfma16(ah, b, c[t]);
          } else {
            c[t] = mfma16(ah, il[t][ks], c[t]);
          }
        }
#pragma unroll
        for (int t = 0; t < NS; ++t) c[t] = mfma16(al, ih[t][ks], c[t]);
      }
      if (nt > 0) {
#pragma unroll
        for (int q = 0; q < NP; ++q)
          if (piece_at(q) == ks) piece(nt - 1, q, pm, pc);
      }
    }
#pragma unroll
    for (int t = 0; t < NS; ++t) { pm[t] = m[t]; pc[t] = c[t]; }
  }
#pragma unroll
  for (int q = 0; q < NP; ++q) piece(NT - 1, q, pm, pc);
}

template <int NS, int KS, class WS>
__device__ __forceinline__ void head22(WS& ws, int pbase, int bias_slot, const u32x4 (&ih)[NS][KS], const u32x4 (&il)[NS][KS],
                                       f32x4 (&out)[NS], int lane) {
  const int g = lane >> 4;
  const float4 b = ws.bias4(bias_slot + 4 * g);
  f32x4 m[NS], c[NS];
  m[0][0] = b.x; m[0][1] = b.y; m[0][2] = b.z; m[0][3] = b.w;
  c[0] = f32x4{0.0f, 0.0f, 0.0f, 0.0f};
#pragma unroll
  for (int t = 1; t < NS; ++t) { m[t] = m[0]; c[t] = c[0]; }
#pragma unroll
  for (int ks = 0; ks < KS; ++ks) {
    const u32x4 ah = __builtin_bit_cast(u32x4, next_frag(ws, 2 * (pbase + ks), lane));
    const u32x4 al = __builtin_bit_cast(u32x4, next_frag(ws, 2 * (pbase + ks) + 1, lane));
    if (NS == 2) {
      m[0] = mfma16(ah, ih[0][ks], m[0]);
      c[0] = mfma16(ah, il[0][ks], c[0]);
      m[1] = mfma16(ah, ih[1][ks], m[1]);
      c[1] = mfma16(ah, il[1][ks], c[1]);
      c[0] = mfma16(al, ih[0][ks], c[0]);
      c[1] = mfma16(al, ih[1][ks], c[1]);
    } else {
#pragma unroll
      for (int t = 0; t < NS; ++t) { m[t] = mfma16(ah, ih[t][ks], m[t]); c[t] = mfma16(ah, il[t][ks], c[t]); }
#pragma unroll
      for (int t = 0; t < NS; ++t) c[t] = mfma16(al, ih[t][ks], c[t]);
    }
  }
#pragma unroll
  for (int s = 0; s < NS; ++s)
#pragma unroll
    for (int i = 0; i < 4; ++i) out[s][i] = __builtin_fmaf(c[s][i], LO_INV, m[s][i]);
}

constexpr int NW22 = 4, NW22_ = NW22;
constexpr int PARK_OFF = RING_LDS_BYTES;
template <int NS> constexpr int park_bytes() { return NS > 2 ? (6 * NS + 4) * 64 * NW22_ * 4 : 0; }
template <int K> __device__ __forceinline__ void lds_put(unsigned addr, float v) {
  asm volatile("ds_write_b32 %0, %1 offset:%2" :: "v"(addr), "v"(v), "i"(1024 * K) : "memory");
}
template <int K> __device__ __forceinline__ float lds_get(unsigned addr) {
  float v;
  asm volatile("ds_read_b32 %0, %1 offset:%2\n\ts_waitcnt lgkmcnt(0)" : "=v"(v) : "v"(addr), "i"(1024 * K) : "memory");
  return v;
}
template <int S> __device__ __forceinline__ void park_put(unsigned park, const float (&p)[3], const float (&d)[3]) {
  lds_put<6 * S + 0>(park, p[0]); lds_put<6 * S + 1>(park, p[1]); lds_put<6 * S + 2>(park, p[2]);
  lds_put<6 * S + 3>(park, d[0]); lds_put<6 * S + 4>(park, d[1]); lds_put<6 * S + 5>(park, d[2]);
}
template <int S, int OFF> __device__ __forceinline__ void park_get(unsigned park, float (&v)[3]) {
  v[0] = lds_get<6 * S + OFF>(park); v[1] = lds_get<6 * S + OFF + 1>(park); v[2] = lds_get<6 * S + OFF + 2>(park);
}
__device__ __forceinline__ void park_put_s(int s, unsigned park, const float (&p)[3], const float (&d)[3]) {
  if (s == 0) park_put<0>(park, p, d); else if (s == 1) park_put<1>(park, p, d); else park_put<2>(park, p, d);
}
template <int OFF> __device__ __forceinline__ void park_get_s(int s, unsigned park, float (&v)[3]) {
  if (s == 0) park_get<0, OFF>(park, v); else if (s == 1) park_get<1, OFF>(park, v); else park_get<2, OFF>(park, v);
}

template <int NS, int MODE, class WS>
__device__ __forceinline__ void tiles22(const FwdArgs& a, WS& ws, int64_t wtile0, int64_t nwtiles, int lane, PassQueue& pq) {
  constexpr bool RECOMP = NS > 2;
  static_assert(!RECOMP || MODE == 1, "the 48-sample form takes rays + depths");
  const int c = lane & 15, g = lane >> 4;
  u32x4 peh[NS][2], pel[NS][2], dph[NS][1], dpl[NS][1];
  const unsigned park = ws.lds0 + PARK_OFF + 4u * (unsigned)(ws.wv * 64 + lane);
  pq.ask(ws.wv, lane);
  const GroupFreq q = group_freqs(a.fr, g);
  {
    const int64_t wt = wtile0 < nwtiles ? wtile0 : nwtiles - 1;
#pragma unroll
    for (int s = 0; s < NS; ++s) {
      const int64_t m = clamp_sample(wt * (16 * NS) + 16 * s + c, a.M);
      if (MODE == 0) {
        row_group<SplitF16, false>(a.x + m * 90, g, peh[s], pel[s]);
        row_group<SplitF16, true>(a.x + m * 90 + 63, g, dph[s], dpl[s]);
      } else {
#if NERF_ABLATE == 3
        Sample sm;
#pragma unroll
        for (int k = 0; k < 3; ++k) { sm.p[k] = 0.001f * (float)(m & 1023) + (float)k; sm.d[k] = 0.5f; }
#else
        const Sample sm = load_sample(a.rays, a.z, m, a.n);
#endif
        if (RECOMP) park_put_s(s, park, sm.p, sm.d);
        encode_group<SinCodyWaite, SplitF16, false>(q, sm.p, peh[s], pel[s]);
        if (!RECOMP) encode_group<SinCodyWaite, SplitF16, true>(q, sm.d, dph[s], dpl[s]);
      }
    }
  }
  pq.publish(ws.wv);
  u32x4 hah[NS][8], hal[NS][8], hbh[NS][8], hbl[NS][8];
  layer22<NS, 2, 16, true>(ws, L16::F_L0, 0, peh, pel, hah, hal, lane);
  layer22<NS, 8, 16, true>(ws, L16::F_L1 + 0 * 128, 256, hah, hal, hbh, hbl, lane);
  layer22<NS, 8, 16, true>(ws, L16::F_L1 + 1 * 128, 512, hbh, hbl, hah, hal, lane);
  layer22<NS, 8, 16, true>(ws, L16::F_L1 + 2 * 128, 768, hah, hal, hbh, hbl, lane);
  layer22<NS, 8, 16, true>(ws, L16::F_L1 + 3 * 128, 1024, hbh, hbl, hah, hal, lane);
  {
    u32x4 cth[NS][10], ctl[NS][10];
#pragma unroll
    for (int s = 0; s < NS; ++s) {
      if (RECOMP) {
        float pp[3];
        park_get_s<0>(s, park, pp);
        encode_group<SinCodyWaite, SplitF16, false>(q, pp, peh[s], pel[s]);
      }
      cth[s][0] = peh[s][0]; cth[s][1] = peh[s][1]; ctl[s][0] = pel[s][0]; ctl[s][1] = pel[s][1];
#pragma unroll
      for (int k = 0; k < 8; ++k) { cth[s][2 + k] = hah[s][k]; ctl[s][2 + k] = hal[s][k]; }
    }
    layer22<NS, 10, 16, true, WS, (NS > 2 ? NERF_F22_PARK : 0)>(ws, L16::F_L5, 1280, cth, ctl, hbh, hbl, lane,
                                            ws.lds0 + PARK_OFF + 6 * NS * 64 * NW22 * 4 + 16u * (unsigned)(ws.wv * 64 + lane), park);
  }
  layer22<NS, 8, 16, true>(ws, L16::F_L6, 1536, hbh, hbl, hah, hal, lane);
  layer22<NS, 8, 16, true>(ws, L16::F_L7, 1792, hah, hal, hbh, hbl, lane);
#if NERF_F22_FOLD
  u32x4 (&fth)[NS][8] = hbh, (&ftl)[NS][8] = hbl;
#else
  layer22<NS, 8, 16, false>(ws, P_FEAT, L::BI_FEAT, hbh, hbl, hah, hal, lane);
  u32x4 (&fth)[NS][8] = hah, (&ftl)[NS][8] = hal;
#endif
  f32x4 alpha[NS];
  head22<NS, 8>(ws, P_ALPHA, L::BI_ALPHA, hbh, hbl, alpha, lane);
  u32x4 hdh[NS][4], hdl[NS][4];
  {
    u32x4 cth[NS][9], ctl[NS][9];
#pragma unroll
    for (int s = 0; s < NS; ++s) {
#pragma unroll
      for (int k = 0; k < 8; ++k) { cth[s][k] = fth[s][k]; ctl[s][k] = ftl[s][k]; }
      if (RECOMP) {
        float dd[3];
        park_get_s<3>(s, park, dd);
        encode_group<SinCodyWaite, SplitF16, true>(q, dd, dph[s], dpl[s]);
      }
      cth[s][8] = dph[s][0]; ctl[s][8] = dpl[s][0];
    }
    layer22<NS, 9, 8, true>(ws, P_DIR, L::BI_DIR, cth, ctl, hdh, hdl, lane);
  }
  f32x4 rgb[NS];
  head22<NS, 4>(ws, P_RGB, L::BI_RGB, hdh, hdl, rgb, lane);
#pragma unroll
  for (int s = 0; s < NS; ++s) {
    const int64_t m = wtile0 * (16 * NS) + 16 * s + c;
    if (g == 0 && wtile0 < nwtiles && m < a.M) {
      float4 o; o.x = rgb[s][0]; o.y = rgb[s][1]; o.z = rgb[s][2]; o.w = alpha[s][0];
      *reinterpret_cast<float4*>(a.out + m * 4) = o;
    }
  }
}

template <int MODE, int NS = 2>
__global__ void __launch_bounds__(64 * NW22) mlp22_fwd_kernel(FwdArgs a) {
  const int lane = threadIdx.x & 63;
  const int wv = __builtin_amdgcn_readfirstlane(threadIdx.x >> 6);
  const int64_t nwtiles = (a.M + 16 * NS - 1) / (16 * NS), nsuper = (nwtiles + NW22 - 1) / NW22;
  NERF_STAMP2_DECL();
  RingW<CHUNKS, F_FRAGS, (NS > 2 ? NERF_F22_RG3 : 4), NW22, RING_CHUNK, RING_STAGES, true, true> ws;
  ws.wsrc = reinterpret_cast<const char*>(a.wf);
  ws.lane16 = 16 * lane;
  ws.lds0 = __builtin_amdgcn_readfirstlane(lds_addr_of(ring_smem));
  ws.wv = wv;
  ws.start(lane);
  ring_load_bias(a.bias, BIAS_FLOATS);
  __syncthreads();
  NERF_STAMP2_LOOP();
  PassQueue pq;
  pq.init(a.queue, ws.lds0 + RING_BIAS_OFF);
  for (int64_t sp = blockIdx.x; sp < nsuper;) {
    int ln = lane;
    asm volatile("" : "+v"(ln));
    ws.new_pass();
    tiles22<NS, MODE>(a, ws, sp * NW22 + wv, nwtiles, ln, pq);
    NERF_STAMP2_PASS();
    sp = pq.next(sp);
  }
  NERF_STAMP2_END();
  ws.drain();
  pq.leave();
}

int pack(const float* params, void* packed22, hipStream_t s) {
  char* base = static_cast<char*>(packed22);
  return launch<pack22_kernel>("nerf_mlp_pack (split-fp16 image)", dim3((PACK_THREADS + 255) / 256), dim3(256), 0, s, params,
                               reinterpret_cast<u32x4*>(base), reinterpret_cast<float*>(base + (size_t)F_PADDED * 1024));
}

int g_tiles = 0;

int forward(const void* packed22, const float* x, const float* rays, const float* z, int64_t M, int n, int freq_mode,
            float* out, int persistent_wgs, hipStream_t s) {
  FwdArgs a;
  a.queue = passq_slot();
  const char* base = static_cast<const char*>(packed22);
  a.wf = reinterpret_cast<const bf16x8*>(base);
  a.bias = reinterpret_cast<const float*>(base + (size_t)F_PADDED * 1024);
  a.x = x; a.rays = rays; a.z = z; a.M = M; a.n = n; a.out = out; a.acts = nullptr; a.astride = 0;
  fill_freqs(a.fr.pos, a.fr.dir, freq_mode);
  int tiles = g_tiles;
  if (tiles == 0) {
    const int64_t w = persistent_wgs > 0 ? persistent_wgs : 1;
    const int64_t p2 = (((M + 31) / 32 + NW22 - 1) / NW22 + w - 1) / w, p3 = (((M + 47) / 48 + NW22 - 1) / NW22 + w - 1) / w;
    tiles = 100 * p2 < 141 * p3 ? 2 : 3;
  }
  return with_index<3>(x ? 0 : (tiles == 3 ? 2 : 1), [&](auto form) {
    constexpr int MODE = decltype(form)::value == 0 ? 0 : 1, NS = decltype(form)::value == 2 ? 3 : 2;
    const int64_t nsuper = ((M + 16 * NS - 1) / (16 * NS) + NW22 - 1) / NW22;
    return launch<mlp22_fwd_kernel<MODE, NS>>("mlp forward (split fp16)", dim3(persistent_grid(nsuper, persistent_wgs)), dim3(64 * NW22),
                                             Lds(RING_LDS_BYTES + park_bytes<NS>(), RING_LDS_BYTES + park_bytes<3>()), s, a);
  });
}

}
}
NERF_STAMP2_EXPORT(nerf_debug_stamps2_mlp22)
```

nerf_meets_mlx_amd/csrc/mlp_index.h:

```cpp
#pragma once
#if !defined(__HIPCC__) && !defined(__host__)
#define __host__
#define __device__
#endif
#include "mlp_params.h"

namespace nerf {

namespace L {
constexpr int F_L0 = 0, F_L1 = 32, F_L5 = 544, F_L6 = 704, F_L7 = 832, F_FA = 960, F_DIR = 1104, F_RGB = 1176;
constexpr int F_TOTAL = 1184;
constexpr int B_RGB = 0, B_DIR = 4, B_FA = 68, B_L7 = 204, B_L6 = 332, B_L5 = 460, B_L4 = 588;
constexpr int B_TOTAL = 1100, B_PADDED = 1120;
constexpr int BI_FEAT = 2048, BI_ALPHA = 2304, BI_DIR = 2336, BI_RGB = 2464, BI_TOTAL = 2496;
}

__host__ __device__ constexpr int kperm(int ks, int h, int j) { return 16 * ks + 8 * (j >> 2) + 4 * h + (j & 3); }
__host__ __device__ constexpr int kperm_ks(int kk) { return kk >> 4; }
__host__ __device__ constexpr int kperm_h(int kk) { return (kk >> 2) & 1; }
__host__ __device__ constexpr int kperm_j(int kk) { return 4 * ((kk >> 3) & 1) + (kk & 3); }

__host__ __device__ constexpr int kperm16(int ks, int g, int j) { return 32 * ks + 16 * (j >> 2) + 4 * g + (j & 3); }
__host__ __device__ constexpr int pos_chan16(int ks, int g, int j) {
  const int sl = 8 * ks + j;
  if (sl < 12) return 3 + 6 * (2 * g + sl / 6) + (sl % 6);
  if (sl < 15) return 3 + 6 * (8 + (g >> 1)) + 3 * (g & 1) + (sl - 12);
  return g < 3 ? g : -1;
}
__host__ __device__ constexpr int dir_chan16(int g, int j) {
  if (j < 6) return 3 + 6 * g + j;
  return (j == 6 && g < 3) ? g : -1;
}

__host__ __device__ constexpr int fwd_index(int f, int r, int h, int j) {
  if (f < L::F_L1) {
    const int nt = f / 4, ks = f % 4;
    const int kk = kperm(ks, h, j);
    return kk < 63 ? L::P_W0 + (32 * nt + r) * 63 + kk : -1;
  }
  if (f < L::F_L5) {
    const int l = 1 + (f - L::F_L1) / 128, g = (f - L::F_L1) % 128;
    const int nt = g / 16, ks = g % 16;
    return L::pw(l) + (32 * nt + r) * 256 + kperm(ks, h, j);
  }
  if (f < L::F_L6) {
    const int g = f - L::F_L5;
    const int nt = g / 20, ks = g % 20;
    const int kk = kperm(ks, h, j), n = 32 * nt + r;
    if (kk < 64) return kk < 63 ? L::P_W5 + n * 319 + kk : -1;
    return L::P_W5 + n * 319 + 63 + (kk - 64);
  }
  if (f < L::F_FA) {
    const int l = 6 + (f - L::F_L6) / 128, g = (f - L::F_L6) % 128;
    const int nt = g / 16, ks = g % 16;
    return L::pw(l) + (32 * nt + r) * 256 + kperm(ks, h, j);
  }
  if (f < L::F_DIR) {
    const int g = f - L::F_FA;
    const int nt = g / 16, ks = g % 16;
    const int kk = kperm(ks, h, j);
    if (nt < 8) return L::P_WF + (32 * nt + r) * 256 + kk;
    return r == 0 ? L::P_WA + kk : -1;
  }
  if (f < L::F_RGB) {
    const int g = f - L::F_DIR;
    const int nt = g / 18, ks = g % 18;
    const int kk = kperm(ks, h, j), n = 32 * nt + r;
    if (kk < 256) return L::P_WD + n * 283 + kk;
    return (kk - 256) < 27 ? L::P_WD + n * 283 + kk : -1;
  }
  const int ks = f - L::F_RGB;
  return r < 3 ? L::P_WR + r * 128 + kperm(ks, h, j) : -1;
}

__host__ __device__ constexpr int bwd_index(int f, int r, int h, int j) {
  if (f < L::B_DIR) {
    const int nn = kperm(0, h, j);
    return nn < 3 ? L::P_WR + nn * 128 + 32 * f + r : -1;
  }
  if (f < L::B_FA) {
    const int g = f - L::B_DIR, kt = g / 8, ns = g % 8;
    return L::P_WD + kperm(ns, h, j) * 283 + 32 * kt + r;
  }
  if (f < L::B_L7) {
    const int g = f - L::B_FA, kt = g / 17, ns = g % 17;
    const int nn = kperm(ns, h, j);
    if (ns < 16) return L::P_WF + nn * 256 + 32 * kt + r;
    return nn == 256 ? L::P_WA + 32 * kt + r : -1;
  }
  const int g = f - L::B_L7, li = g / 128, q = g % 128, kt = q / 16, ns = q % 16;
  const int l = 7 - li, nn = kperm(ns, h, j), row = 32 * kt + r;
  if (l == 5) return L::P_W5 + nn * 319 + 63 + row;
  return L::pw(l) + nn * 256 + row;
}

namespace LF {
constexpr int F_A = L::F_FA, F_DIR = F_A + 16, F_RGB = F_DIR + 72, F_TOTAL = F_RGB + 8;
constexpr int B_RGB = 0, B_DA = 4, B_L7 = B_DA + 72, B_TOTAL = B_L7 + 7 * 128;
constexpr int B_PADDED = 976;
constexpr int B_SHIFT = L::B_L7 - B_L7;
constexpr int C_WFT = 2 * F_TOTAL * 256, C_WFT_END = C_WFT + 256 * 256;
constexpr int C_WD1 = (2 * L::F_TOTAL + 2 * B_PADDED) * 256, C_BF = C_WD1 + 128 * 256, C_BP = C_BF + 256, C_USED = C_BP + 128;
constexpr int C_END = (2 * L::F_TOTAL + 2 * 1104) * 256;
static_assert(C_WFT_END == 2 * L::F_TOTAL * 256, "W_F^T fills the forward stream's freed fragments exactly");
static_assert(C_USED <= C_END, "the copies fit the transposed stream's freed fragments");
}
__host__ __device__ constexpr int fold_wp(int n, int k) { return -2 - (n * 256 + k); }
__host__ __device__ constexpr bool is_fold_wp(int src) { return src <= -2; }
__host__ __device__ constexpr int fold_wp_n(int src) { return (-2 - src) >> 8; }
__host__ __device__ constexpr int fold_wp_k(int src) { return (-2 - src) & 255; }

__host__ __device__ constexpr int fwd_index_fold(int f, int r, int h, int j) {
  if (f < LF::F_A) return fwd_index(f, r, h, j);
  if (f < LF::F_DIR) return r == 0 ? L::P_WA + kperm(f - LF::F_A, h, j) : -1;
  if (f < LF::F_RGB) {
    const int g = f - LF::F_DIR;
    const int nt = g / 18, ks = g % 18;
    const int kk = kperm(ks, h, j), n = 32 * nt + r;
    if (kk < 256) return fold_wp(n, kk);
    return (kk - 256) < 27 ? L::P_WD + n * 283 + kk : -1;
  }
  const int ks = f - LF::F_RGB;
  return r < 3 ? L::P_WR + r * 128 + kperm(ks, h, j) : -1;
}
__host__ __device__ constexpr int bwd_index_fold(int f, int r, int h, int j) {
  if (f < LF::B_DA) return bwd_index(f, r, h, j);
  if (f < LF::B_L7) {
    const int g = f - LF::B_DA, kt = g / 9, ns = g % 9;
    const int nn = kperm(ns, h, j), row = 32 * kt + r;
    if (ns < 8) return fold_wp(nn, row);
    return nn == 128 ? L::P_WA + row : -1;
  }
  return bwd_index(f + LF::B_SHIFT, r, h, j);
}

__host__ __device__ constexpr int bias_index(int s) {
  if (s < L::BI_FEAT) return L::pb(s >> 8) + (s & 255);
  if (s < L::BI_ALPHA) return L::P_BF + (s - L::BI_FEAT);
  if (s < L::BI_DIR) return s == L::BI_ALPHA ? L::P_BA : -1;
  if (s < L::BI_RGB) return L::P_BD + (s - L::BI_DIR);
  return (s - L::BI_RGB) < 3 ? L::P_BR + (s - L::BI_RGB) : -1;
}
struct ViewPack {
  static constexpr int F_TOTAL = L::F_TOTAL, F_PADDED = L::F_TOTAL, B_TOTAL = L::B_TOTAL, B_PADDED = L::B_PADDED, BI_TOTAL = L::BI_TOTAL;
  static __host__ __device__ constexpr int fwd(int f, int r, int h, int j, int) { return fwd_index(f, r, h, j); }
  static __host__ __device__ constexpr int bwd(int f, int r, int h, int j, int) { return bwd_index(f, r, h, j); }
  static __host__ __device__ constexpr int bias(int s, int) { return bias_index(s); }
};
template <class S>
__host__ __device__ constexpr int pack_index(bool fw, int f, int r, int h, int j, int out_ch) {
  if (f >= (fw ? S::F_TOTAL : S::B_TOTAL)) return -1;
  return fw ? S::fwd(f, r, h, j, out_ch) : S::bwd(f, r, h, j, out_ch);
}

struct FragElem { int f, r, h, j; };
__host__ __device__ constexpr FragElem fwd_elem_feature(int row, int col) {
  return FragElem{L::F_FA + 16 * (row >> 5) + kperm_ks(col), row & 31, kperm_h(col), kperm_j(col)};
}
__host__ __device__ constexpr FragElem fwd_elem_dir0(int row, int col) {
  return FragElem{L::F_DIR + 18 * (row >> 5) + kperm_ks(col), row & 31, kperm_h(col), kperm_j(col)};
}
__host__ __device__ constexpr FragElem fold_elem_fwd(int n, int k) {
  return FragElem{LF::F_DIR + 18 * (n >> 5) + kperm_ks(k), n & 31, kperm_h(k), kperm_j(k)};
}
__host__ __device__ constexpr FragElem fold_elem_bwd(int n, int k) {
  return FragElem{LF::B_DA + 9 * (k >> 5) + kperm_ks(n), k & 31, kperm_h(n), kperm_j(n)};
}
__host__ __device__ constexpr int frag_elem_offset(const FragElem& e) { return (e.f * 64 + 32 * e.h + e.r) * 8 + e.j; }

}
```

nerf_meets_mlx_amd/csrc/mlp_s16.h:

```cpp
#pragma once
#include <hip/hip_runtime.h>
#include <stdint.h>

namespace nerf {
struct DwArgs;
namespace s16 {

constexpr int A_LO = 158, A_MASK = 316, A_SLOTS = 325;
constexpr int Z_LO = 154, Z_SLOTS = 308;
constexpr int F_FRAGS = 2368, B_FRAGS = 2200, B_PADDED = 2208;
constexpr int64_t PACKED_BYTES = (int64_t)(F_FRAGS + B_PADDED) * 1024;

int pack(const float* params, void* packed_s16, bool fold, hipStream_t s);
int forward(const void* packed_s16, const float* bias_slots, const float* x, const float* rays, const float* z, int64_t M,
            int n, int freq_mode, float* out, void* acts, int64_t astride16, int persistent_wgs, bool fold, hipStream_t s);
int backward_chain(const void* packed_s16, const void* acts, const float* d_raw, int64_t M, void* dz, int64_t astride16,
                   int64_t zstride16, int persistent_wgs, bool fold, hipStream_t s);
int pack_folded(const float* params, void* packed_s16, hipStream_t s);
int forward_folded(const void* packed_s16, const float* bias_slots, const float* x, const float* rays, const float* z, int64_t M,
                   int n, int freq_mode, float* out, void* acts, int64_t astride16, int persistent_wgs, hipStream_t s);
int backward_chain_folded(const void* packed_s16, const void* acts, const float* d_raw, int64_t M, void* dz, int64_t astride16,
                          int64_t zstride16, int persistent_wgs, hipStream_t s);
int launch_dw_kernel(const DwArgs& d, int workgroups, bool split_bf16, hipStream_t s);
extern int g_dw_variant;

}
}
```

nerf_meets_mlx_amd/csrc/mlp_s16.hip:

```cpp
#include "mlp_s16_view.h"
#include "mlp_pack.h"

namespace nerf {
namespace s16 {

struct ViewPairPack : ViewPack { static constexpr int B_PADDED = s16::B_PADDED / 2; };
static_assert(ViewPairPack::B_PADDED >= L::B_TOTAL, "the padded stream holds every transposed fragment");

#ifndef NERF_DWX
#define NERF_DWX 0
#endif
#if NERF_DWX & 4
#define DW_BARRIER() do {} while (0)
#else
#define DW_BARRIER() __builtin_amdgcn_s_barrier()
#endif
constexpr int DW_WAVES = 16, DW_NPW = 2;

__device__ __forceinline__ bf16x8 tr_pair(const char* blk, int hq, int fsel, int i16) {
  const int q = i16 >> 2, p = i16 & 3;
  const char* base = blk + 64 * (8 * hq + q) + 32 * fsel + 16 * (p & 1) + 8 * (p >> 1);
#if NERF_DWX & 2
  bf16x8 r; asm volatile("" : "=v"(r) : "v"(base)); return r;
#endif
// ... 160 lines not shown
      default: break;
    }
  }
  const bool active = (wr * DW_NPW < n_tiles) && (wc * 2 < k_tiles);
  const int kc = (k_tiles + 1) >> 1;
  int stride = npairs * 1024, ns = DW_LDS_BYTES / stride;
  if (ns > a.ring_cap) ns = a.ring_cap;
  const int cnt_w = (wv < npairs ? 1 : 0) + (wv + DW_WAVES < npairs ? 1 : 0);
  f32x16 acc[DW_NPW][2];
#pragma unroll
  for (int i = 0; i < DW_NPW; ++i)
#pragma unroll
    for (int k = 0; k < 2; ++k)
#pragma unroll
      for (int e = 0; e < 16; ++e) acc[i][k][e] = 0.0f;
  float bsum[2 * DW_NPW];
  bool own[2 * DW_NPW];
#pragma unroll
  for (int c = 0; c < 2 * DW_NPW; ++c) { bsum[c] = 0.0f; own[c] = (c % kc) == wc && !(NERF_DWX & 8); }
  const int g16 = lane >> 4, i16 = lane & 15, hq = g16 >> 1, fsel = g16 & 1;
  const unsigned lds0 = __builtin_amdgcn_readfirstlane(lds_addr_of(smem));
  const int src_row = lane >> 2, src_sel = (lane >> 1) & 1, src_half = lane & 1;
  const char* dzb = reinterpret_cast<const char*>(a.dz);
  const char* acb = reinterpret_cast<const char*>(a.acts);
  long long zstride_b = a.zstride * 16, astride_b = a.astride * 16;
  int z_lo = a.z_lo, a_lo = a.a_lo, dz_slot = jb.dz_slot, act_slot = jb.act_slot, nf = jb.nf, kf = jb.kf;
  asm volatile("" : "+s"(zstride_b), "+s"(astride_b), "+s"(z_lo), "+s"(a_lo), "+s"(dz_slot), "+s"(act_slot), "+s"(nf), "+s"(kf),
               "+s"(stride), "+s"(ns));

  auto issue = [&](int ht, int slot) {
#if NERF_DWX & 1
    return;
#endif
    const unsigned st = lds0 + __builtin_amdgcn_readfirstlane(slot) * stride;
    const int64_t tile = SPLIT ? ht >> 1 : ht;
    const unsigned row_off0 = (unsigned)(32 * ((SPLIT ? 16 * (ht & 1) : 0) + src_row) + 16 * src_half);
#pragma unroll
    for (int k = 0; k < DW_NPW; ++k) {
      const int i = wv + DW_WAVES * k;
      if (i < npairs) {
        const bool is_z = i < 2 * n_tiles;
        const int j = is_z ? i : i - 2 * n_tiles;
        const int nt_ = is_z ? n_tiles : k_tiles;
        const int lo_part = j >= nt_ ? 1 : 0;
        const int t = lo_part ? j - nt_ : j;
        const int nfr = is_z ? nf : kf;
        int fr = 2 * t + src_sel; if (fr >= nfr) fr = nfr - 1;
        const int slot_ = (is_z ? dz_slot + (SPLIT ? lo_part * z_lo : 0) : act_slot + (SPLIT ? lo_part * a_lo : 0)) + fr;
        const unsigned row_off = row_off0 + (SPLIT ? 0 : 512 * lo_part);
        const char* src = (is_z ? dzb + tile * zstride_b : acb + tile * astride_b) + (int64_t)slot_ * 1024 + row_off;
        dma_frag_nt(src, st + i * 1024);
      }
    }
  };
  auto process = [&](const char* st) {
    if (active) {
      bf16x8 bh[2], bl[2];
#pragma unroll
      for (int k = 0; k < 2; ++k) {
        const int kt = wc * 2 + k;
        const int b = 2 * n_tiles + (kt < k_tiles ? kt : 0);
        bh[k] = tr_pair(st + b * 1024, hq, fsel, i16);
        bl[k] = tr_pair(st + (b + k_tiles) * 1024, hq, fsel, i16);
      }
#pragma unroll
      for (int i = 0; i < DW_NPW; ++i) {
        const int nt = wr * DW_NPW + i;
        const int b = nt < n_tiles ? nt : 0;
        const bf16x8 ah = tr_pair(st + b * 1024, hq, fsel, i16);
        const bf16x8 al = tr_pair(st + (b + n_tiles) * 1024, hq, fsel, i16);
        const bf16x2 ones = {(__bf16)1.0f, (__bf16)1.0f};
        if (own[2 * i]) {
          asm volatile("" ::: "memory");
#pragma unroll
          for (int j = 0; j < 8; j += 2) { const bf16x2 q = {ah[j], ah[j + 1]}; bsum[2 * i] = __builtin_amdgcn_fdot2_f32_bf16(q, ones, bsum[2 * i], false); }
        }
        if (own[2 * i + 1]) {
          asm volatile("" ::: "memory");
#pragma unroll
          for (int j = 0; j < 8; j += 2) { const bf16x2 q = {al[j], al[j + 1]}; bsum[2 * i + 1] = __builtin_amdgcn_fdot2_f32_bf16(q, ones, bsum[2 * i + 1], false); }
        }
#if NERF_DWX & 16
        asm volatile("" :: "v"(ah), "v"(al), "v"(bh[0]), "v"(bl[0]), "v"(bh[1]), "v"(bl[1]));
#else
#pragma unroll
        for (int k = 0; k < 2; ++k) {
          if (SPLIT) {
            acc[i][k] = mfma32(al, bh[k], acc[i][k]);
            acc[i][k] = mfma32(ah, bl[k], acc[i][k]);
            acc[i][k] = mfma32(ah, bh[k], acc[i][k]);
          } else {
            acc[i][k] = mfma32(ah, bh[k], acc[i][k]);
            acc[i][k] = mfma32(al, bl[k], acc[i][k]);
          }
        }
#endif
      }
    }
  };
  auto wait_landed = [&](int younger) {
    switch (younger * cnt_w) {
#define NERF_VM_CASE(N) case N: asm volatile("s_waitcnt vmcnt(" #N ") lgkmcnt(0)" ::: "memory"); break;
      NERF_VM_CASE(0) NERF_VM_CASE(1) NERF_VM_CASE(2) NERF_VM_CASE(3) NERF_VM_CASE(4) NERF_VM_CASE(5) NERF_VM_CASE(6) NERF_VM_CASE(7)
      NERF_VM_CASE(8) NERF_VM_CASE(9) NERF_VM_CASE(10) NERF_VM_CASE(11) NERF_VM_CASE(12) NERF_VM_CASE(13) NERF_VM_CASE(14)
      NERF_VM_CASE(16) NERF_VM_CASE(18) NERF_VM_CASE(20) NERF_VM_CASE(22) NERF_VM_CASE(24) NERF_VM_CASE(26) NERF_VM_CASE(28)
#undef NERF_VM_CASE
      default: asm volatile("s_waitcnt vmcnt(0) lgkmcnt(0)" ::: "memory"); break;
    }
  };
  const int ht_lo = SPLIT ? 2 * tile_lo : tile_lo, n = SPLIT ? 2 * (tile_hi - tile_lo) : tile_hi - tile_lo;
  int issued = 0, slot_i = 0, slot_p = 0;
  for (; issued < ns && issued < n; ++issued) { issue(ht_lo + issued, slot_i); slot_i = slot_i + 1 == ns ? 0 : slot_i + 1; }
  for (int p = 0; p < n; p += 2) {
    wait_landed(issued - (p + 2 < n ? p + 2 : n));
    DW_BARRIER();
#pragma unroll
    for (int k = 0; k < 2; ++k)
      if (issued < n && issued - ns < p) { issue(ht_lo + issued, slot_i); slot_i = slot_i + 1 == ns ? 0 : slot_i + 1; ++issued; }
    process(smem + slot_p * stride); slot_p = slot_p + 1 == ns ? 0 : slot_p + 1;
    if (SPLIT || p + 1 < n) { process(smem + slot_p * stride); slot_p = slot_p + 1 == ns ? 0 : slot_p + 1; }
  }
  asm volatile("s_waitcnt lgkmcnt(0)" ::: "memory");
  __builtin_amdgcn_s_barrier();
  float* xb = reinterpret_cast<float*>(smem);
#pragma unroll
  for (int c = 0; c < 2 * DW_NPW; ++c)
    if (own[c] && active) xb[(wr * 2 * DW_NPW + c) * 64 + lane] = bsum[c];
  __builtin_amdgcn_s_barrier();
  if (!active) return;
  const int rr = lane & 31, hh = lane >> 5;
  float* slot = a.partial + (size_t)blockIdx.x * DW_SLOT_FLOATS;
#pragma unroll
  for (int i = 0; i < DW_NPW; ++i) {
    const int nt = wr * DW_NPW + i;
    if (nt >= n_tiles) continue;
#pragma unroll
    for (int k = 0; k < 2; ++k) {
      const int kt = wc * 2 + k;
      if (kt >= k_tiles) continue;
      float* tile = slot + (8 * nt + kt) * 1024;
#pragma unroll
      for (int e = 0; e < 16; ++e) tile[((e & 3) + 8 * (e >> 2) + 4 * hh) * 32 + rr] = acc[i][k][e];
    }
    if (wc == 0 && jb.b_off >= 0) {
      const float lo = xb[(wr * 2 * DW_NPW + 2 * i + 1) * 64 + lane], hi = xb[(wr * 2 * DW_NPW + 2 * i) * 64 + lane];
      const float t = lo + hi;
      const float tot = t + __shfl_xor(t, 32, 64);
      if (hh == 0) slot[64 * 1024 + 32 * nt + rr] = tot;
    }
  }
}


int pack(const float* params, void* packed_s16, bool fold, hipStream_t s) {
  bf16x8* wf = static_cast<bf16x8*>(packed_s16);
  if (fold) return pack_folded(params, packed_s16, s);
  return launch<pack_streams_kernel<ViewPairPack, SplitBf16, false>>("nerf_mlp_pack (split-bf16 image)", dim3(pack_blocks<ViewPairPack, false>()),
                                                                     dim3(256), 0, s, params, wf, wf + (size_t)F_FRAGS * 64, nullptr, 0);
}

int forward(const void* packed_s16, const float* bias_slots, const float* x, const float* rays, const float* z, int64_t M,
            int n, int freq_mode, float* out, void* acts, int64_t astride16, int persistent_wgs, bool fold, hipStream_t s) {
  if (fold)
    return forward_folded(packed_s16, bias_slots, x, rays, z, M, n, freq_mode, out, acts, astride16, persistent_wgs, s);
  FwdArgs a;
  a.queue = passq_slot();
  a.wf = reinterpret_cast<const bf16x8*>(packed_s16);
  a.bias = bias_slots;
  a.x = x; a.rays = rays; a.z = z; a.M = M; a.n = n; a.out = out; a.acts = acts; a.astride = astride16;
  fill_freqs(a.fr.pos, a.fr.dir, freq_mode);
  const int64_t nsuper = ((M + 31) / 32 + NW - 1) / NW;
  return with_bool(x != nullptr, [&](auto rows) {
    return launch<s16_fwd_kernel<decltype(rows)::value ? 0 : 1, false>>("mlp training forward (split bf16)", dim3(persistent_grid(nsuper, persistent_wgs)),
                                                                         dim3(64 * NW), FwdRing::LDS_BYTES, s, a);
  });
}

int backward_chain(const void* packed_s16, const void* acts, const float* d_raw, int64_t M, void* dz, int64_t astride16,
                   int64_t zstride16, int persistent_wgs, bool fold, hipStream_t s) {
  if (fold) return backward_chain_folded(packed_s16, acts, d_raw, M, dz, astride16, zstride16, persistent_wgs, s);
  BwdArgs b;
  b.queue = passq_slot();
  b.wb = reinterpret_cast<const bf16x8*>(static_cast<const char*>(packed_s16) + (size_t)F_FRAGS * 1024);
  b.acts = acts; b.d_raw = d_raw; b.M = M; b.dz = dz; b.astride = astride16; b.zstride = zstride16;
  const int64_t nsuper = ((M + 31) / 32 + NW - 1) / NW;
  return launch<s16_bwd_kernel<false>>("mlp backward chain (split bf16)", dim3(persistent_grid(nsuper, persistent_wgs)), dim3(64 * NW),
                                       BwdRing::LDS_BYTES, s, b);
}

int g_dw_variant = 1;

int launch_dw_kernel(const DwArgs& d, int workgroups, bool split_bf16, hipStream_t s) {
  return with_bool(split_bf16, [&](auto split) {
    return launch<s16_dw_kernel<decltype(split)::value>>(split_bf16 ? "mlp dW (split bf16)" : "mlp dW (bf16)", dim3(workgroups), dim3(64 * DW_WAVES),
                                                         DW_LDS_BYTES, s, d);
  });
}

}
}
```

nerf_meets_mlx_amd/csrc/mlp_s16f.hip:

```cpp
#include "mlp_s16_view.h"

namespace nerf {
namespace s16 {

constexpr int FOLD_PACK_PAIRS = (LF::F_TOTAL + LF::B_PADDED) * 64;
constexpr int FOLD_PACK_THREADS = FOLD_PACK_PAIRS + (LF::C_WFT_END - LF::C_WFT) + (LF::C_END - LF::C_WD1);
__global__ void __launch_bounds__(256) pack_fold_kernel(const float* __restrict__ p, bf16x8* __restrict__ img) {
  const int tid = blockIdx.x * 256 + threadIdx.x;
  bf16x8* wf = img;
  bf16x8* wb = img + (size_t)F_FRAGS * 64;
  float* cp = reinterpret_cast<float*>(img);
  if (tid < FOLD_PACK_PAIRS) {
    const bool fw = tid < LF::F_TOTAL * 64;
    const int t = fw ? tid : tid - LF::F_TOTAL * 64;
    const int f = t >> 6, lane = t & 63, r = lane & 31, h = lane >> 5;
    int src[8];
#pragma unroll
    for (int j = 0; j < 8; ++j) src[j] = !fw && f >= LF::B_TOTAL ? -1 : fw ? fwd_index_fold(f, r, h, j) : bwd_index_fold(f, r, h, j);
    const bool wp = is_fold_wp(src[0]);
    if (wp && !fw) return;
    float v[8];
    if (wp) {
      const int n = fold_wp_n(src[0]);
      double acc[8];
#pragma unroll
      for (int j = 0; j < 8; ++j) acc[j] = 0.0;
      for (int q = 0; q < 256; ++q) {
        const double wd = (double)p[L::P_WD + n * 283 + q];
#pragma unroll
        for (int j = 0; j < 8; ++j) acc[j] = __builtin_fma(wd, (double)p[L::P_WF + q * 256 + fold_wp_k(src[j])], acc[j]);
      }
#pragma unroll
      for (int j = 0; j < 8; ++j) v[j] = (float)acc[j];
    } else {
#pragma unroll
      for (int j = 0; j < 8; ++j) v[j] = src[j] >= 0 ? p[src[j]] : 0.0f;
    }
    bf16x8 o[2];
    SplitBf16::pack(v, o[0], o[1]);
    bf16x8* dst = fw ? wf : wb;
    dst[(2 * f) * 64 + lane] = o[0];
    dst[(2 * f + 1) * 64 + lane] = o[1];
    if (wp) {
      __bf16* tb = reinterpret_cast<__bf16*>(wb);
#pragma unroll
      for (int j = 0; j < 8; ++j) {
        const FragElem e = fold_elem_bwd(fold_wp_n(src[j]), fold_wp_k(src[j]));
        FragElem eh = e, el = e;
        eh.f = 2 * e.f; el.f = 2 * e.f + 1;
        tb[frag_elem_offset(eh)] = o[0][j];
        tb[frag_elem_offset(el)] = o[1][j];
      }
    }
    return;
  }
  int c = tid - FOLD_PACK_PAIRS;
  if (c < LF::C_WFT_END - LF::C_WFT) {
    cp[LF::C_WFT + c] = p[L::P_WF + (c & 255) * 256 + (c >> 8)];
    return;
  }
  c += LF::C_WD1 - (LF::C_WFT_END - LF::C_WFT);
  if (c >= LF::C_END) return;
  float v = 0.0f;
  if (c < LF::C_BF) { const int e = c - LF::C_WD1; v = p[L::P_WD + (e >> 8) * 283 + (e & 255)]; }
  else if (c < LF::C_BP) v = p[L::P_BF + (c - LF::C_BF)];
  else if (c < LF::C_USED) {
    const int n = c - LF::C_BP;
    double acc = 0.0;
    for (int q = 0; q < 256; ++q) acc = __builtin_fma((double)p[L::P_WD + n * 283 + q], (double)p[L::P_BF + q], acc);
    v = (float)(acc + (double)p[L::P_BD + n]);
  }
  cp[c] = v;
}

int pack_folded(const float* params, void* packed_s16, hipStream_t s) {
  return launch<pack_fold_kernel>("nerf_mlp_pack (split-bf16 image, folded)", dim3((FOLD_PACK_THREADS + 255) / 256), dim3(256), 0, s, params,
                                  static_cast<bf16x8*>(packed_s16));
}

int forward_folded(const void* packed_s16, const float* bias_slots, const float* x, const float* rays, const float* z, int64_t M,
                   int n, int freq_mode, float* out, void* acts, int64_t astride16, int persistent_wgs, hipStream_t s) {
  FwdArgs a;
  a.queue = passq_slot();
  a.wf = reinterpret_cast<const bf16x8*>(packed_s16);
  a.bias = bias_slots;
  a.x = x; a.rays = rays; a.z = z; a.M = M; a.n = n; a.out = out; a.acts = acts; a.astride = astride16;
  fill_freqs(a.fr.pos, a.fr.dir, freq_mode);
  const int64_t nsuper = ((M + 31) / 32 + NW - 1) / NW;
  return with_bool(x != nullptr, [&](auto rows) {
    return launch<s16_fwd_kernel<decltype(rows)::value ? 0 : 1, true>>("mlp training forward (split bf16, folded)",
                                                                        dim3(persistent_grid(nsuper, persistent_wgs)), dim3(64 * NW),
                                                                        FwdRingFold::LDS_BYTES, s, a);
  });
}

int backward_chain_folded(const void* packed_s16, const void* acts, const float* d_raw, int64_t M, void* dz, int64_t astride16,
                          int64_t zstride16, int persistent_wgs, hipStream_t s) {
  BwdArgs b;
  b.queue = passq_slot();
  b.wb = reinterpret_cast<const bf16x8*>(static_cast<const char*>(packed_s16) + (size_t)F_FRAGS * 1024);
  b.acts = acts; b.d_raw = d_raw; b.M = M; b.dz = dz; b.astride = astride16; b.zstride = zstride16;
  const int64_t nsuper = ((M + 31) / 32 + NW - 1) / NW;
  return launch<s16_bwd_kernel<true>>("mlp backward chain (split bf16, folded)", dim3(persistent_grid(nsuper, persistent_wgs)), dim3(64 * NW),
                                      BwdRingFold::LDS_BYTES, s, b);
}

}
}
```

nerf_meets_mlx_amd/csrc/sampling.hip:

```cpp
#include "launch.h"

namespace nerf {

__device__ __forceinline__ float jitter_z(float v, int k, int n, float below, float above, float t, float s) {
  const float lo = (k == 0) ? v : 0.5f * (below + v);
  const float hi = (k == n - 1) ? v : 0.5f * (v + above);
  return lo + (hi - lo) * (t * s);
}

__global__ void sample_coarse_kernel(const float* __restrict__ rays, int64_t B, int n, int lindisp, float perturb,
                                     const float* __restrict__ t_rand, float step, float* __restrict__ z) {
  const int64_t total = B * n;
  for (int64_t t = blockIdx.x * (int64_t)blockDim.x + threadIdx.x; t < total; t += (int64_t)gridDim.x * blockDim.x) {
    const int64_t b = t / n; const int k = (int)(t - b * n);
    const float near = rays[b * NERF_RAY_STRIDE + 6], far = rays[b * NERF_RAY_STRIDE + 7];
    auto zk = [&](int kk) -> float {
      const float tv = (float)kk * step + 0.0f;
      if (!lindisp) return near * (1.0f - tv) + far * tv;
      return 1.0f / (1.0f / (near * (1.0f - tv)) + 1.0f / (far * tv));
    };
    float v = zk(k);
    if (perturb > 0.0f) v = jitter_z(v, k, n, k == 0 ? v : zk(k - 1), k == n - 1 ? v : zk(k + 1), t_rand[t], perturb);
    z[t] = v;
  }
}

__global__ void add_noise_z_kernel(const float* __restrict__ z_in, const float* __restrict__ t_rand, int64_t B, int n,
                                   float strength, float* __restrict__ z_out) {
  const int64_t total = B * n;
  for (int64_t t = blockIdx.x * (int64_t)blockDim.x + threadIdx.x; t < total; t += (int64_t)gridDim.x * blockDim.x) {
    const int k = (int)(t % n);
    const float v = z_in[t];
    z_out[t] = jitter_z(v, k, n, k == 0 ? v : z_in[t - 1], k == n - 1 ? v : z_in[t + 1], t_rand[t], strength);
  }
}

template <int CH>
__global__ void __launch_bounds__(256) importance_kernel(const float* __restrict__ z, const float* __restrict__ w,
                                                         const float* __restrict__ u, int64_t B, int n, int N,
                                                         int P, float eps, float* __restrict__ z_new,
                                                         float* __restrict__ z_merged, float* __restrict__ cdf_out,
                                                         int64_t* __restrict__ inds_out) {
  extern __shared__ __attribute__((aligned(16))) float smem[];
  const int lane = threadIdx.x & 63, wv = threadIdx.x >> 6;
  const int per_wave = (n + 1) * 2 + ((n + P + 3) & ~3);
  float* s_cdf = smem + wv * per_wave;
  float* s_zmid = s_cdf + (n + 1);
  float* s_all = s_zmid + (n + 1);
  for (int64_t ray = blockIdx.x * 4 + wv; ray < B; ray += (int64_t)gridDim.x * 4) {
    const float* zr = z + ray * n;
    const float* wr = w + ray * n;
    float wl[CH];
    double part = 0.0;
#pragma unroll
    for (int c = 0; c < CH; ++c) {
      const int k = lane * CH + c;
      wl[c] = (k < n) ? wr[k] + 0.01f : 0.0f;
      part += (double)wl[c];
    }
    float s = (float)wave_sum(part);
    const float pad = fmaxf(eps - s, 0.0f);
    const float padw = pad / (float)n;
    s = s + pad;
    double run = 0.0;
    double loc[CH];
#pragma unroll
    for (int c = 0; c < CH; ++c) {
      const int k = lane * CH + c;
      const float pdf = (k < n) ? (wl[c] + padw) / s : 0.0f;
      run += (double)pdf;
      loc[c] = run;
    }
    const double incl = wave_scan_incl(run, lane);
    const double excl = incl - run;
    if (lane == 0) s_cdf[0] = 0.0f;
#pragma unroll
    for (int c = 0; c < CH; ++c) {
      const int k = lane * CH + c;
      if (k < n) s_cdf[k + 1] = fminf(1.0f, (float)(excl + loc[c]));
    }
    for (int i = lane; i <= n; i += WAVE) {
      int a = i - 1; a = a < 0 ? 0 : (a > n - 2 ? n - 2 : a);
      s_zmid[i] = (zr[a + 1] + zr[a]) / 2.0f;
    }
    for (int i = lane; i < n; i += WAVE) s_all[i] = zr[i];
    __builtin_amdgcn_s_waitcnt(0);
    __builtin_amdgcn_wave_barrier();
    if (cdf_out) for (int i = lane; i <= n; i += WAVE) cdf_out[ray * (n + 1) + i] = s_cdf[i];
    bool new_nan = false;
    for (int j = lane; j < N; j += WAVE) {
      const float uj = u[ray * N + j];
      const bool unan = uj != uj;
      int lo = 0, hi = n + 1;
      while (lo < hi) { const int mid = (lo + hi) >> 1; if (unan || s_cdf[mid] <= uj) lo = mid + 1; else hi = mid; }
      const int inds = lo;
      int below = inds - 1; below = below < 0 ? 0 : (below > n ? n : below);
      int above = inds;     above = above > n ? n : above;
      const float cf = s_cdf[below], ct = s_cdf[above];
      const float zf = s_zmid[below], zt = s_zmid[above];
      float den = ct - cf;
      den = (den < eps) ? 1.0f : den;
      float t = (uj - cf) / den;
      if (t != t) t = 0.0f;
      t = fminf(fmaxf(t, 0.0f), 1.0f);
      const float zn = zf + t * (zt - zf);
      new_nan = new_nan || (zn != zn);
      if (z_new) z_new[ray * N + j] = zn;
      if (inds_out) inds_out[ray * N + j] = inds;
      s_all[n + j] = zn;
    }
    __builtin_amdgcn_s_waitcnt(0);
    __builtin_amdgcn_wave_barrier();
    if (z_merged) {
      const int tot = n + N;
      float* s_new = s_all + n;
      bool asc = !new_nan;
      for (int i = lane; i + 1 < n; i += WAVE) asc = asc && (s_all[i] <= s_all[i + 1]);
      if (__all(asc)) {
        for (int i = N + lane; i < P; i += WAVE) s_new[i] = __builtin_inff();
        __builtin_amdgcn_s_waitcnt(0);
        __builtin_amdgcn_wave_barrier();
        for (int k = 2; k <= P; k <<= 1) {
          for (int j = k >> 1; j > 0; j >>= 1) {
            for (int pi = lane; pi < (P >> 1); pi += WAVE) {
              const int i = ((pi & ~(j - 1)) << 1) | (pi & (j - 1));
              const int q = i | j;
              const float a = s_new[i], b = s_new[q];
              const bool up = (i & k) == 0;
              if ((a > b) == up) { s_new[i] = b; s_new[q] = a; }
            }
            __builtin_amdgcn_s_waitcnt(0);
            __builtin_amdgcn_wave_barrier();
          }
        }
        for (int i = lane; i < n; i += WAVE) {
          const float v = s_all[i];
          int lo = 0, hi = N;
          while (lo < hi) { const int mid = (lo + hi) >> 1; if (s_new[mid] < v) lo = mid + 1; else hi = mid; }
          z_merged[ray * tot + i + lo] = v;
        }
        for (int j = lane; j < N; j += WAVE) {
          const float v = s_new[j];
          int lo = 0, hi = n;
          while (lo < hi) { const int mid = (lo + hi) >> 1; if (s_all[mid] <= v) lo = mid + 1; else hi = mid; }
          z_merged[ray * tot + j + lo] = v;
        }
      } else {
        for (int i = lane; i < tot; i += WAVE) {
          const float v = s_all[i];
          int rank = 0;
          for (int k = 0; k < tot; ++k) {
            const float o = s_all[k];
            const bool less = (o < v) || (v != v && o == o) || ((o == v || (o != o && v != v)) && k < i);
            rank += less ? 1 : 0;
          }
          z_merged[ray * tot + rank] = v;
        }
      }
    }
    __builtin_amdgcn_s_waitcnt(0);
    __builtin_amdgcn_wave_barrier();
  }
}

}

using namespace nerf;

extern "C" int nerf_sample_coarse(const float* rays, int64_t B, int n, int lindisp, float perturb,
                                  const float* t_rand, float* z, void* stream) {
  NERF_REQUIRE(B >= 0 && n >= 2, NERF_E_SHAPE, "nerf_sample_coarse: need n >= 2 (n=%d)", n);
  if (B == 0) return NERF_OK;
  NERF_REQUIRE(rays && z, NERF_E_NULL, "nerf_sample_coarse: rays/z is NULL");
  NERF_REQUIRE(perturb <= 0.0f || t_rand, NERF_E_NULL, "nerf_sample_coarse: perturb > 0 needs t_rand");
  const float step = (float)((1.0 - 0.0) / (double)(n - 1));
  NERF_LAUNCH("nerf_sample_coarse", sample_coarse_kernel, grid_for(B * n, 256), 256, as_stream(stream), rays, B, n, lindisp,
              perturb, t_rand, step, z);
  return NERF_OK;
}

extern "C" int nerf_add_noise_z(const float* z_in, const float* t_rand, int64_t B, int n, float strength, float* z_out,
                               void* stream) {
  NERF_REQUIRE(B >= 0 && n >= 1, NERF_E_SHAPE, "nerf_add_noise_z: bad B/n");
  if (B == 0) return NERF_OK;
  NERF_REQUIRE(z_in && t_rand && z_out, NERF_E_NULL, "nerf_add_noise_z: NULL pointer");
  NERF_REQUIRE(z_in != z_out, NERF_E_SHAPE, "nerf_add_noise_z: in-place use is not supported (neighbours are read)");
  NERF_LAUNCH("nerf_add_noise_z", add_noise_z_kernel, grid_for(B * n, 256), 256, as_stream(stream), z_in, t_rand, B, n, strength,
              z_out);
  return NERF_OK;
}

extern "C" int nerf_importance_sample(const float* z, const float* weights, const float* u, int64_t B, int n, int N,
                                      float eps, float* z_new, float* z_merged, float* cdf, int64_t* inds,
                                      void* stream) {
  NERF_REQUIRE(n >= 2 && n <= 256 && N >= 1 && N <= 512 && n + N <= 768, NERF_E_SHAPE,
               "nerf_importance_sample: unsupported n=%d N=%d (2<=n<=256, 1<=N<=512)", n, N);
  if (B <= 0) return NERF_OK;
  NERF_REQUIRE(z && weights && u, NERF_E_NULL, "nerf_importance_sample: z/weights/u is NULL");
  int P = 2;
  while (P < N) P <<= 1;
  const int per_wave = (n + 1) * 2 + ((n + P + 3) & ~3);
  const int lds = per_wave * 4 * (int)sizeof(float);
  return with_int_up_to<1, 2, 3, 4>((n + 63) / 64, [&](auto ch) {
    return launch<importance_kernel<decltype(ch)::value>>("nerf_importance_sample", dim3(wave_per_ray_grid(B, 256 * 8)), dim3(256),
                                                          lds, as_stream(stream), z, weights, u, B, n, N, P, eps, z_new, z_merged,
                                                          cdf, inds);
  });
}
```

nerf_meets_mlx_amd/models/NeRF.py:

```python
import contextlib
import ctypes as C
import math
from typing import Dict, List, Optional

import numpy as np
import torch

from .. import _native as N
from . import embedding

_LAYERS = None


def layer_shapes(n_layers=8, width=256, cin=63, cdir=27, skips=(4,), use_viewdirs=True, cout=4):
    s = [("pos0", width, cin)]
    for i in range(n_layers - 1):
        s.append((f"pos{i + 1}", width, width + cin if i in skips else width))
    if use_viewdirs:
        s += [("feature", width, width), ("alpha", 1, width), ("dir0", width // 2, width + cdir), ("rgb", 3, width // 2)]
    else:
        s += [("output", cout, width)]
    return s


class NeRF:

    def __init__(self, n_layers=8, width_layers=256, channel_input=3, channel_input_views=3, channel_output=4,
                 list_skip_connection_layers=[4], is_use_view_directions=False, device="cuda", seed: Optional[int] = None,
                 precision: int = 22):
        self.D, self.W = n_layers, width_layers
        self.channel_input_pos, self.channel_input_dir = channel_input, channel_input_views
        self.list_skip_connection_layers = list(list_skip_connection_layers)
        self.is_use_view_directions = is_use_view_directions
        self.device = torch.device(device)
        self.shapes = layer_shapes(n_layers, width_layers, channel_input, channel_input_views,
                                   tuple(self.list_skip_connection_layers), is_use_view_directions, channel_output)
        self.n_params = sum(o * i + o for _, o, i in self.shapes)
        self.arch = N.MlpArch(n_layers, width_layers, channel_input, channel_input_views,
                              self.list_skip_connection_layers[0] if len(self.list_skip_connection_layers) == 1 else -1,
                              int(bool(is_use_view_directions)), channel_output, int(precision))
        if precision not in (16, 22, 32):
            raise ValueError("NeRF: precision must be 16 (bf16 MFMA operands), 32 (fp32 MFMA) or 22 (float32 tolerance on the "
                             "16-bit matrix pipe: split-bf16 training, split-fp16 inference)")
        self.precision = int(precision)
        self.out_dim = 4 if is_use_view_directions else channel_output
        rng = np.random.default_rng(seed)
        chunks = []
        for _, o, i in self.shapes:
            k = 1.0 / math.sqrt(i)
            chunks.append(rng.uniform(-k, k, size=(o, i)).astype(np.float32).reshape(-1))
            chunks.append(rng.uniform(-k, k, size=(o,)).astype(np.float32))
        self.params = torch.from_numpy(np.concatenate(chunks)).to(self.device)
        self.grads = torch.zeros_like(self.params)
        self._packed = None
        self._dirty = True
        self._packed_version = -1
        self._ws: Dict[str, torch.Tensor] = {}
        self.name: Optional[str] = None
        self._gen = 0
        self._acts_gen = -1
        self._acts_M = -1
        self.train_fold = False
        self._packed_form = 0
        self._acts_form = 0
        self._can_fold = (precision == 22 and bool(is_use_view_directions) and n_layers == 8 and width_layers == 256
                          and channel_input == 63 and channel_input_views == 27 and self.list_skip_connection_layers == [4])

    def parameters(self) -> Dict[str, object]:
        views, off = {}, 0
        for name, o, i in self.shapes:
            views[name] = {"weight": self.params[off:off + o * i].view(o, i), "bias": self.params[off + o * i:off + o * i + o]}
            off += o * i + o
        tree = {"list_linears_pos": [views[f"pos{l}"] for l in range(self.D)]}
        if self.is_use_view_directions:
            tree.update({"list_linears_dir": [views["dir0"]], "feature_linear": views["feature"],
                         "alpha_linear": views["alpha"], "rgb_linear": views["rgb"]})
        else:
            tree["output_linear"] = views["output"]
        return tree

    def trainable(self) -> torch.Tensor:
        if not self.params.requires_grad:
            self.params.requires_grad_(True)
        return self.params

    def load_flat(self, flat: torch.Tensor):
        assert flat.numel() == self.n_params
        with torch.no_grad():
            self.params.copy_(flat.to(self.device, torch.float32).reshape(-1))
        self._dirty = True

    def mark_updated(self):
        self._dirty = True

    def activation_generation(self) -> int:
        return self._acts_gen

    def train_form(self) -> int:
        if not (self.train_fold and self._can_fold):
            return 0
        lib = N.lib()
        return int(lib.nerf_get_option(b"train_fold") in (0, 1) and lib.nerf_get_option(b"dw_factor") == 1
                   and lib.nerf_get_option(b"dw22_variant") != 0 and lib.nerf_get_option(b"dw_job_mask") == 0)

    @contextlib.contextmanager
    def _form(self, form: int):
        if not self._can_fold:
            yield
            return
        lib = N.lib()
        before = lib.nerf_get_option(b"train_fold")
        if before not in (0, 1):
            yield
            return
        N.check(lib.nerf_set_option(b"train_fold", int(form)))
        try:
            yield
        finally:
            lib.nerf_set_option(b"train_fold", before)

    def packed(self) -> torch.Tensor:
        lib = N.lib()
        if self._packed is None:
            nbytes = lib.nerf_mlp_packed_bytes(C.byref(self.arch))
            if nbytes < 0:
                raise ValueError("libnerf_hip error -3: this NeRF architecture / precision has no HIP kernel (supported: "
                                 "n_layers=8, width=256, skips=[4] with in=63+27 + view head [precision 16, 22, 32], or in=40 without "
                                 "view head and out<=4 [16, 22, 32]; n_layers=2, width=64, skips=[] with in=32+16 + view head [16, 22])")
            self._packed = torch.empty(nbytes, dtype=torch.uint8, device=self.device)
        form = self.train_form()
        if self._dirty or self.params._version != self._packed_version or form != self._packed_form:
            with self._form(form):
                N.check(lib.nerf_mlp_pack(C.byref(self.arch), N.ptr(self.params), N.ptr(self._packed), N.stream()))
            self._dirty = False
            self._packed_version = self.params._version
            self._packed_form = form
        return self._packed

    def _begin_train_pass(self, M: int) -> torch.Tensor:
        acts = self._workspace("acts", N.lib().nerf_mlp_acts_bytes(C.byref(self.arch), M))
        self._gen += 1
        self._acts_gen, self._acts_M = self._gen, M
        return acts

    def _workspace(self, key: str, nbytes: int) -> torch.Tensor:
        t = self._ws.get(key)
        if t is None or t.numel() < nbytes:
            t = torch.empty(nbytes, dtype=torch.uint8, device=self.device)
            self._ws[key] = t
        return t

    def forward(self, x: torch.Tensor, train: bool = False) -> torch.Tensor:
        x = N.f32(x).reshape(-1, x.shape[-1])
        M = x.shape[0]
        out = torch.empty(M, self.out_dim, dtype=torch.float32, device=x.device)
        acts = None
        if train:
            acts = self._begin_train_pass(M)
        packed = self.packed()
        with self._form(self._packed_form):
            N.check(N.lib().nerf_mlp_forward_train(C.byref(self.arch), N.ptr(packed), N.ptr(x), M, N.ptr(out),
                                                   N.ptr(acts), N.stream()))
        if train:
            self._acts_form = self._packed_form
        return out

    __call__ = forward

    def query(self, rays: torch.Tensor, z: torch.Tensor, ref_quirks: bool = True, train: bool = False) -> torch.Tensor:
        B, n = z.shape
        raw = torch.empty(B, n, 4, dtype=torch.float32, device=z.device)
        acts = None
        if train:
            acts = self._begin_train_pass(B * n)
        packed = self.packed()
        with self._form(self._packed_form):
            N.check(N.lib().nerf_query_fused(C.byref(self.arch), N.ptr(packed), N.ptr(rays), N.ptr(z), B, n,
                                             0 if ref_quirks else 1, N.ptr(raw), N.ptr(acts), N.stream()))
        if train:
            self._acts_form = self._packed_form
        return raw

    def backward(self, d_raw: torch.Tensor, need_input_grad: bool = False, generation: Optional[int] = None):
        d_raw = N.f32(d_raw)
        M = d_raw.numel() // self.out_dim
        if generation is not None and generation != self._acts_gen:
            raise RuntimeError(f"NeRF.backward: the activations of forward #{generation} were overwritten by train-mode "
                               f"forward #{self._acts_gen} of the same model (one activation workspace per model: run "
                               "backward before the next train-mode forward, or use a second model object)")
        assert M == self._acts_M, "backward() needs a matching query/forward(train=True) first"
        dz = self._workspace("dz", N.lib().nerf_mlp_dz_bytes(C.byref(self.arch), M))
        packed = self.packed()
        if self._packed_form != getattr(self, "_acts_form", 0):
            raise RuntimeError("NeRF.backward: the training form (train_fold / the options it depends on) changed between the "
                               "train-mode forward and backward; run the forward again")
        if need_input_grad:
            d_x = torch.empty(M, self.channel_input_pos, dtype=torch.float32, device=d_raw.device)
            N.check(N.lib().nerf_mlp_backward_inputs(C.byref(self.arch), N.ptr(self.packed()), N.ptr(self._ws["acts"]),
                                                     N.ptr(d_raw), M, N.ptr(dz), N.ptr(self.grads), N.ptr(d_x), N.stream()))
            return self.grads, d_x
        with self._form(self._packed_form):
            N.check(N.lib().nerf_mlp_backward(C.byref(self.arch), N.ptr(packed), N.ptr(self._ws["acts"]),
                                              N.ptr(d_raw), M, N.ptr(dz), N.ptr(self.grads), N.stream()))
        return self.grads


def debug_layer(model: NeRF, kind: str, layer: int) -> torch.Tensor:
    k = {"acts": 0, "dz": 1}[kind]
    if layer == 8 and getattr(model, "_acts_form", 0):
        raise ValueError("debug_layer: a folded model (train_fold) neither computes nor stores the feature layer's activations and "
                         "dZ (layer 8): its dir0 reads h7 through W' = W_D[:, :256] W_F")
    w = N.lib().nerf_mlp_debug_width(C.byref(model.arch), k, layer)
    if w < 0:
        raise ValueError("debug_layer: no such (kind, layer) in this model's training stores (include/nerf_hip.h, nerf_mlp_debug_read)")
    M = model._acts_M
    out = torch.empty(M, w, dtype=torch.float32, device=model.device)
    N.check(N.lib().nerf_mlp_debug_read(C.byref(model.arch), N.ptr(model._ws[kind]), k, layer, M, N.ptr(out), N.stream()))
    return out


class Adam:

    def __init__(self, learning_rate: float, betas=(0.9, 0.999), eps: float = 1e-8, bias_correction: bool = False,
                 shared_state: bool = True):
        self.learning_rate = learning_rate
        self.betas, self.eps = betas, eps
        self.bias_correction, self.shared_state = bias_correction, shared_state
        self.state: Dict[str, List[torch.Tensor]] = {}
        self.step_count: Dict[str, int] = {}
        self._auto_names: Dict[int, str] = {}

    def key_of(self, model) -> str:
        if self.shared_state:
            return "shared"
        name = getattr(model, "name", None)
        if name:
            return str(name)
        return self._auto_names.setdefault(id(model), f"model{len(self._auto_names)}")

    def update(self, model: NeRF, grads: Optional[torch.Tensor] = None, grad_scale: float = 1.0, zero_grads: bool = False):
        g = model.grads if grads is None else grads
        key = self.key_of(model)
        if key not in self.state:
            self.state[key] = [torch.zeros_like(model.params), torch.zeros_like(model.params)]
        self.step_count[key] = self.step_count.get(key, 0) + 1
        m, v = self.state[key]
        half = getattr(model, "half", None)
        if zero_grads or g.dtype == torch.int64 or half is not None:
            N.check(N.lib().nerf_adam_step_shadow(N.ptr(model.params), N.ptr(g), N.ptr(m), N.ptr(v), model.n_params,
                                                  float(self.learning_rate), float(self.betas[0]), float(self.betas[1]),
                                                  float(self.eps), int(self.bias_correction), self.step_count[key],
                                                  float(grad_scale), int(g.dtype == torch.int64), int(bool(zero_grads)),
                                                  N.ptr(half), N.stream()))
            if half is not None:
                model.mark_updated(shadow_written=True)
                return
        else:
            N.check(N.lib().nerf_adam_step(N.ptr(model.params), N.ptr(g), N.ptr(m), N.ptr(v), model.n_params,
                                           float(self.learning_rate), float(self.betas[0]), float(self.betas[1]),
                                           float(self.eps), int(self.bias_correction), self.step_count[key],
                                           float(grad_scale), N.stream()))
        model.mark_updated()

    def update_spans(self, model, spans, grad_scale: float = 1.0):
        key = self.key_of(model)
        if key not in self.state:
            self.state[key] = [torch.zeros_like(model.params), torch.zeros_like(model.params)]
        self.step_count[key] = self.step_count.get(key, 0) + 1
        m, v = self.state[key]
        half = getattr(model, "half", None)
        for lo, hi, g in spans:
            assert g.numel() == hi - lo and g.is_contiguous()
            N.check(N.lib().nerf_adam_step_shadow(N.ptr(model.params[lo:hi]), N.ptr(g), N.ptr(m[lo:hi]), N.ptr(v[lo:hi]), hi - lo,
                                                  float(self.learning_rate), float(self.betas[0]), float(self.betas[1]),
                                                  float(self.eps), int(self.bias_correction), self.step_count[key],
                                                  float(grad_scale), int(g.dtype == torch.int64), 0,
                                                  N.ptr(half[lo:hi]) if half is not None else None, N.stream()))
        model.mark_updated()

    def state_dict(self) -> Dict[str, object]:
        return {"state": {k: [t.detach().cpu() for t in v] for k, v in self.state.items()},
                "step_count": dict(self.step_count), "learning_rate": float(self.learning_rate)}

    def load_state_dict(self, sd, device="cuda"):
        self.state = {k: [t.to(device, torch.float32).contiguous().clone() for t in v] for k, v in sd["state"].items()}
        self.step_count = {k: int(v) for k, v in sd.get("step_count", {}).items()}
# ... 61 lines not shown
```

Baseline: 1.396 million.

## Compute folded feature-layer product once and add register bitonic importance merge

Adds a fold kernel that computes the view-direction-by-feature weight product and folded bias once per parameter generation, and lets both the fp16 and bf16 pack kernels read that buffer. Before this, each pack recomputed the double-precision 256-long dot products inside every pack kernel. It also adds a register-resident bitonic sort plus a merge-by-rank path for importance sampling that writes the merged z row through LDS. The trade-offs are an extra buffer and an extra launch, plus more kernel template instantiations.

```diff
diff --git a/include/nerf_hip.h b/include/nerf_hip.h
--- a/include/nerf_hip.h
+++ b/include/nerf_hip.h
@@ -121,6 +121,9 @@
 int64_t nerf_mlp_param_count(const nerf_mlp_arch* arch);
 int64_t nerf_mlp_packed_bytes(const nerf_mlp_arch* arch);
 int nerf_mlp_pack(const nerf_mlp_arch* arch, const float* params, void* packed, void* stream);
+#define NERF_MLP_FOLD_FLOATS (128 * 256 + 128)
+int nerf_mlp_fold(const nerf_mlp_arch* arch, const float* params, float* fold, void* stream);
+int nerf_mlp_pack_fold(const nerf_mlp_arch* arch, const float* params, const float* fold, void* packed, void* stream);
 
 int64_t nerf_mlp_acts_bytes(const nerf_mlp_arch* arch, int64_t M);
 int64_t nerf_mlp_dz_bytes(const nerf_mlp_arch* arch, int64_t M);
diff --git a/nerf_meets_mlx_amd/_native.py b/nerf_meets_mlx_amd/_native.py
--- a/nerf_meets_mlx_amd/_native.py
+++ b/nerf_meets_mlx_amd/_native.py
@@ -43,6 +43,8 @@
     "nerf_mlp_param_count": (_I64, [_P]),
     "nerf_mlp_packed_bytes": (_I64, [_P]),
     "nerf_mlp_pack": (_I, [_P, _P, _P, _P]),
+    "nerf_mlp_fold": (_I, [_P, _P, _P, _P]),
+    "nerf_mlp_pack_fold": (_I, [_P, _P, _P, _P, _P]),
     "nerf_mlp_acts_bytes": (_I64, [_P, _I64]),
     "nerf_mlp_dz_bytes": (_I64, [_P, _I64]),
     "nerf_mlp_forward": (_I, [_P, _P, _P, _I64, _P, _P]),
@@ -146,6 +148,10 @@
 }
 
 
+_SINCE_FOLD_ONCE = ("nerf_mlp_fold", "nerf_mlp_pack_fold")
+FOLD_FLOATS = 128 * 256 + 128
+
+
 class MlpArch(C.Structure):
     _fields_ = [("n_layers", _I), ("width", _I), ("in_pos", _I), ("in_dir", _I), ("skip_layer", _I),
                 ("use_viewdirs", _I), ("out_ch", _I), ("precision", _I)]
@@ -167,6 +173,8 @@
                 "(hipcc --offload-arch=gfx950).  There is no CPU fallback.")
         L = C.CDLL(LIB_PATH)
         for name, (res, args) in SIGNATURES.items():
+            if name in _SINCE_FOLD_ONCE and "NERF_HIP_LIB" in os.environ and not hasattr(L, name):
+                continue
             fn = getattr(L, name)
             fn.restype, fn.argtypes = res, args
         _lib = L
diff --git a/nerf_meets_mlx_amd/csrc/mlp.hip b/nerf_meets_mlx_amd/csrc/mlp.hip
--- a/nerf_meets_mlx_amd/csrc/mlp.hip
+++ b/nerf_meets_mlx_amd/csrc/mlp.hip
@@ -16,6 +16,7 @@
 namespace nerf {
 
 extern int g_hash_combine_max_res;
+extern int g_importance_variant;
 
 
 
@@ -1108,6 +1109,7 @@
 static int g_dw_narrow_first = 1;
 static int g_dw_factor = 1;
 static int g_train_fold = 0;
+static int g_fold_once = 1;
 static int g_dw_job_mask = 0;
 static int g_mlp_variant = 0;
 static int g_ring_wgs = 0;
@@ -1154,6 +1156,8 @@
     {"dw_narrow_first", &g_dw_narrow_first, opt_flag, nullptr},
     {"dw_factor", &g_dw_factor, opt_flag, nullptr},
     {"train_fold", &g_train_fold, opt_flag, nullptr},
+    {"fold_once", &g_fold_once, opt_flag, nullptr},
+    {"importance_variant", &g_importance_variant, opt_flag, nullptr},
     {"f22_tiles", &f22::g_tiles, [](int& v) { return v == 0 || v == 2 || v == 3; }, "nerf_set_option: f22_tiles must be 0 (automatic), 2 or 3"},
 };
 
@@ -1191,9 +1195,49 @@
   const Model m = resolve(arch); \
   NERF_REQUIRE(m.ok, NERF_E_UNSUPPORTED, who NERF_ARCH_MSG)
 
+namespace nerf {
+__global__ void __launch_bounds__(64) fold_kernel(const float* __restrict__ p, float* __restrict__ fold) {
+  const int t = blockIdx.x * 64 + threadIdx.x;
+  if (t < FOLD_WP_FLOATS) {
+    const float* __restrict__ wd = p + L::P_WD + (blockIdx.x >> 2) * 283;
+    const float* __restrict__ wf = p + L::P_WF + (t & 255);
+    double acc = 0.0;
+#pragma unroll 64
+    for (int f = 0; f < 256; ++f) acc = __builtin_fma((double)wd[f], (double)wf[f * 256], acc);
+    fold[t] = (float)acc;
+  } else if (t < FOLD_FLOATS) {
+    const int n = t - FOLD_WP_FLOATS;
+    const float* __restrict__ wd = p + L::P_WD + n * 283;
+    double acc = 0.0;
+#pragma unroll 16
+    for (int f = 0; f < 256; ++f) acc = __builtin_fma((double)wd[f], (double)p[L::P_BF + f], acc);
+    fold[t] = (float)(acc + (double)p[L::P_BD + n]);
+  }
+}
+static_assert(FOLD_FLOATS == NERF_MLP_FOLD_FLOATS, "fold buffer size of the C ABI");
+}
+
+extern "C" int nerf_mlp_fold(const nerf_mlp_arch* arch, const float* params, float* fold, void* stream) {
+  NERF_RESOLVE("nerf_mlp_fold");
+  NERF_REQUIRE(m.shape == Shape::View && m.split(), NERF_E_UNSUPPORTED, "nerf_mlp_fold: only the 8 x 256 view model at precision 22 folds its feature layer");
+  NERF_REQUIRE(params && fold, NERF_E_NULL, "nerf_mlp_fold: params/fold is NULL");
+  return launch<fold_kernel>("nerf_mlp_fold", dim3((FOLD_FLOATS + 63) / 64), dim3(64), 0, as_stream(stream), params, fold);
+}
+
+static int pack_image(const nerf_mlp_arch* arch, const float* params, const float* fold, void* packed, void* stream, const char* who);
+
 extern "C" int nerf_mlp_pack(const nerf_mlp_arch* arch, const float* params, void* packed, void* stream) {
-  NERF_RESOLVE("nerf_mlp_pack");
-  NERF_REQUIRE(params && packed, NERF_E_NULL, "nerf_mlp_pack: params/packed is NULL");
+  return pack_image(arch, params, nullptr, packed, stream, "nerf_mlp_pack");
+}
+
+extern "C" int nerf_mlp_pack_fold(const nerf_mlp_arch* arch, const float* params, const float* fold, void* packed, void* stream) {
+  return pack_image(arch, params, g_fold_once ? fold : nullptr, packed, stream, "nerf_mlp_pack_fold");
+}
+
+static int pack_image(const nerf_mlp_arch* arch, const float* params, const float* fold, void* packed, void* stream, const char* who) {
+  const Model m = resolve(arch);
+  if (!m.ok) return fail(NERF_E_UNSUPPORTED, "%s%s", who, NERF_ARCH_MSG);
+  if (!params || !packed) return fail(NERF_E_NULL, "%s: params/packed is NULL", who);
   auto s = as_stream(stream);
   bf16x8* wf = m.stream<bf16x8>(packed, S_FWD);
   bf16x8* wb = m.stream<bf16x8>(packed, S_BWD);
@@ -1212,8 +1256,8 @@
     rc = launch<pack_kernel>("nerf_mlp_pack", dim3(PACK_BLOCKS + PACK16_BLOCKS), dim3(256), 0, s, params, wf, wb, bias,
                              m.stream<bf16x8>(packed, S_FWD16));
     if (!rc && m.prec == Prec::F32) rc = f32::pack(params, m.stream<void>(packed, S_F32), 0, s);
-    if (!rc && m.split()) rc = f22::pack(params, m.stream<void>(packed, S_F22), s);
-    if (!rc && m.split()) rc = s16::pack(params, m.stream<void>(packed, S_S16), train_folded(m), s);
+    if (!rc && m.split()) rc = f22::pack(params, fold, m.stream<void>(packed, S_F22), s);
+    if (!rc && m.split()) rc = s16::pack(params, fold, m.stream<void>(packed, S_S16), train_folded(m), s);
   }
   return rc;
 }
diff --git a/nerf_meets_mlx_amd/csrc/mlp22.h b/nerf_meets_mlx_amd/csrc/mlp22.h
--- a/nerf_meets_mlx_amd/csrc/mlp22.h
+++ b/nerf_meets_mlx_amd/csrc/mlp22.h
@@ -54,7 +54,7 @@
 
 #ifdef __HIPCC__
 extern int g_tiles;
-int pack(const float* params, void* packed22, hipStream_t s);
+int pack(const float* params, const float* fold, void* packed22, hipStream_t s);
 int forward(const void* packed22, const float* x, const float* rays, const float* z, int64_t M, int n, int freq_mode,
             float* out, int persistent_wgs, hipStream_t s);
 #endif
diff --git a/nerf_meets_mlx_amd/csrc/mlp22.hip b/nerf_meets_mlx_amd/csrc/mlp22.hip
--- a/nerf_meets_mlx_amd/csrc/mlp22.hip
+++ b/nerf_meets_mlx_amd/csrc/mlp22.hip
@@ -51,7 +51,7 @@
 }
 
 constexpr int PACK_THREADS = (F_PADDED / 2) * 64 + BIAS_FLOATS;
-__global__ void __launch_bounds__(256) pack22_kernel(const float* __restrict__ p, u32x4* __restrict__ wf,
+__global__ void __launch_bounds__(256) pack22_kernel(const float* __restrict__ p, const float* __restrict__ fb, u32x4* __restrict__ wf,
                                                      float* __restrict__ bias) {
   const int t = blockIdx.x * 256 + threadIdx.x;
   if (t < (F_PADDED / 2) * 64) {
@@ -60,7 +60,7 @@
     if (fp < F_PAIRS) {
 #if NERF_F22_FOLD
       float fold[8] = {0.0f, 0.0f, 0.0f, 0.0f, 0.0f, 0.0f, 0.0f, 0.0f};
-      if (fp >= P_DIR && fp < P_RGB && (fp - P_DIR) % 9 < 8) {
+      if (!fb && fp >= P_DIR && fp < P_RGB && (fp - P_DIR) % 9 < 8) {
         const float* __restrict__ wd = p + L::P_WD + (16 * ((fp - P_DIR) / 9) + (lane & 15)) * 283;
         const float* __restrict__ wfk = p + L::P_WF + kperm16((fp - P_DIR) % 9, lane >> 4, 0);
         double acc[8] = {0.0, 0.0, 0.0, 0.0, 0.0, 0.0, 0.0, 0.0};
@@ -82,7 +82,7 @@
         for (int e = 0; e < 2; ++e) {
 #if NERF_F22_FOLD
           const Src src = stream_src(fp, lane & 15, lane >> 4, j + e);
-          w[e] = src.p >= 0 ? p[src.p] : src.p == SRC_FOLD ? fold[j + e] : 0.0f;
+          w[e] = src.p >= 0 ? p[src.p] : src.p == SRC_FOLD ? (fb ? fb[src.n * 256 + src.k] : fold[j + e]) : 0.0f;
 #else
           w[e] = fwd_src16(p, fp, lane & 15, lane >> 4, j + e);
 #endif
@@ -103,6 +103,7 @@
 #if NERF_F22_FOLD
     else if (s < L::BI_ALPHA) v = 0.0f;
     else if (s < L::BI_DIR) v = (s == L::BI_ALPHA) ? p[L::P_BA] : 0.0f;
+    else if (s < L::BI_RGB && fb) v = fb[FOLD_WP_FLOATS + (s - L::BI_DIR)];
     else if (s < L::BI_RGB) {
       const float* __restrict__ wd = p + L::P_WD + (s - L::BI_DIR) * 283;
       double acc = 0.0;
@@ -405,9 +406,9 @@
   pq.leave();
 }
 
-int pack(const float* params, void* packed22, hipStream_t s) {
+int pack(const float* params, const float* fold, void* packed22, hipStream_t s) {
   char* base = static_cast<char*>(packed22);
-  return launch<pack22_kernel>("nerf_mlp_pack (split-fp16 image)", dim3((PACK_THREADS + 255) / 256), dim3(256), 0, s, params,
+  return launch<pack22_kernel>("nerf_mlp_pack (split-fp16 image)", dim3((PACK_THREADS + 255) / 256), dim3(256), 0, s, params, fold,
                                reinterpret_cast<u32x4*>(base), reinterpret_cast<float*>(base + (size_t)F_PADDED * 1024));
 }
 
diff --git a/nerf_meets_mlx_amd/csrc/mlp_index.h b/nerf_meets_mlx_amd/csrc/mlp_index.h
--- a/nerf_meets_mlx_amd/csrc/mlp_index.h
+++ b/nerf_meets_mlx_amd/csrc/mlp_index.h
@@ -109,6 +109,7 @@
 __host__ __device__ constexpr bool is_fold_wp(int src) { return src <= -2; }
 __host__ __device__ constexpr int fold_wp_n(int src) { return (-2 - src) >> 8; }
 __host__ __device__ constexpr int fold_wp_k(int src) { return (-2 - src) & 255; }
+constexpr int FOLD_WP_FLOATS = 128 * 256, FOLD_FLOATS = FOLD_WP_FLOATS + 128;
 
 __host__ __device__ constexpr int fwd_index_fold(int f, int r, int h, int j) {
   if (f < LF::F_A) return fwd_index(f, r, h, j);
diff --git a/nerf_meets_mlx_amd/csrc/mlp_s16.h b/nerf_meets_mlx_amd/csrc/mlp_s16.h
--- a/nerf_meets_mlx_amd/csrc/mlp_s16.h
+++ b/nerf_meets_mlx_amd/csrc/mlp_s16.h
@@ -11,12 +11,12 @@
 constexpr int F_FRAGS = 2368, B_FRAGS = 2200, B_PADDED = 2208;
 constexpr int64_t PACKED_BYTES = (int64_t)(F_FRAGS + B_PADDED) * 1024;
 
-int pack(const float* params, void* packed_s16, bool fold, hipStream_t s);
+int pack(const float* params, const float* wp, void* packed_s16, bool fold, hipStream_t s);
 int forward(const void* packed_s16, const float* bias_slots, const float* x, const float* rays, const float* z, int64_t M,
             int n, int freq_mode, float* out, void* acts, int64_t astride16, int persistent_wgs, bool fold, hipStream_t s);
 int backward_chain(const void* packed_s16, const void* acts, const float* d_raw, int64_t M, void* dz, int64_t astride16,
                    int64_t zstride16, int persistent_wgs, bool fold, hipStream_t s);
-int pack_folded(const float* params, void* packed_s16, hipStream_t s);
+int pack_folded(const float* params, const float* wp, void* packed_s16, hipStream_t s);
 int forward_folded(const void* packed_s16, const float* bias_slots, const float* x, const float* rays, const float* z, int64_t M,
                    int n, int freq_mode, float* out, void* acts, int64_t astride16, int persistent_wgs, hipStream_t s);
 int backward_chain_folded(const void* packed_s16, const void* acts, const float* d_raw, int64_t M, void* dz, int64_t astride16,
diff --git a/nerf_meets_mlx_amd/csrc/mlp_s16.hip b/nerf_meets_mlx_amd/csrc/mlp_s16.hip
--- a/nerf_meets_mlx_amd/csrc/mlp_s16.hip
+++ b/nerf_meets_mlx_amd/csrc/mlp_s16.hip
@@ -336,9 +336,9 @@
 }
 
 
-int pack(const float* params, void* packed_s16, bool fold, hipStream_t s) {
+int pack(const float* params, const float* wp, void* packed_s16, bool fold, hipStream_t s) {
   bf16x8* wf = static_cast<bf16x8*>(packed_s16);
-  if (fold) return pack_folded(params, packed_s16, s);
+  if (fold) return pack_folded(params, wp, packed_s16, s);
   return launch<pack_streams_kernel<ViewPairPack, SplitBf16, false>>("nerf_mlp_pack (split-bf16 image)", dim3(pack_blocks<ViewPairPack, false>()),
                                                                      dim3(256), 0, s, params, wf, wf + (size_t)F_FRAGS * 64, nullptr, 0);
 }
diff --git a/nerf_meets_mlx_amd/csrc/mlp_s16f.hip b/nerf_meets_mlx_amd/csrc/mlp_s16f.hip
--- a/nerf_meets_mlx_amd/csrc/mlp_s16f.hip
+++ b/nerf_meets_mlx_amd/csrc/mlp_s16f.hip
@@ -5,7 +5,7 @@
 
 constexpr int FOLD_PACK_PAIRS = (LF::F_TOTAL + LF::B_PADDED) * 64;
 constexpr int FOLD_PACK_THREADS = FOLD_PACK_PAIRS + (LF::C_WFT_END - LF::C_WFT) + (LF::C_END - LF::C_WD1);
-__global__ void __launch_bounds__(256) pack_fold_kernel(const float* __restrict__ p, bf16x8* __restrict__ img) {
+__global__ void __launch_bounds__(256) pack_fold_kernel(const float* __restrict__ p, const float* __restrict__ fb, bf16x8* __restrict__ img) {
   const int tid = blockIdx.x * 256 + threadIdx.x;
   bf16x8* wf = img;
   bf16x8* wb = img + (size_t)F_FRAGS * 64;
@@ -20,7 +20,10 @@
     const bool wp = is_fold_wp(src[0]);
     if (wp && !fw) return;
     float v[8];
-    if (wp) {
+    if (wp && fb) {
+#pragma unroll
+      for (int j = 0; j < 8; ++j) v[j] = fb[-2 - src[j]];
+    } else if (wp) {
       const int n = fold_wp_n(src[0]);
       double acc[8];
 #pragma unroll
@@ -64,6 +67,7 @@
   float v = 0.0f;
   if (c < LF::C_BF) { const int e = c - LF::C_WD1; v = p[L::P_WD + (e >> 8) * 283 + (e & 255)]; }
   else if (c < LF::C_BP) v = p[L::P_BF + (c - LF::C_BF)];
+  else if (c < LF::C_USED && fb) v = fb[FOLD_WP_FLOATS + (c - LF::C_BP)];
   else if (c < LF::C_USED) {
     const int n = c - LF::C_BP;
     double acc = 0.0;
@@ -73,8 +77,8 @@
   cp[c] = v;
 }
 
-int pack_folded(const float* params, void* packed_s16, hipStream_t s) {
-  return launch<pack_fold_kernel>("nerf_mlp_pack (split-bf16 image, folded)", dim3((FOLD_PACK_THREADS + 255) / 256), dim3(256), 0, s, params,
+int pack_folded(const float* params, const float* wp, void* packed_s16, hipStream_t s) {
+  return launch<pack_fold_kernel>("nerf_mlp_pack (split-bf16 image, folded)", dim3((FOLD_PACK_THREADS + 255) / 256), dim3(256), 0, s, params, wp,
                                   static_cast<bf16x8*>(packed_s16));
 }
 
diff --git a/nerf_meets_mlx_amd/csrc/sampling.hip b/nerf_meets_mlx_amd/csrc/sampling.hip
--- a/nerf_meets_mlx_amd/csrc/sampling.hip
+++ b/nerf_meets_mlx_amd/csrc/sampling.hip
@@ -35,7 +35,52 @@
   }
 }
 
-template <int CH>
+int g_importance_variant = 1;
+
+__device__ __forceinline__ float lane_xor(float v, int j) {
+  const int x = __builtin_bit_cast(int, v);
+  int o;
+  switch (j) {
+    case 1: o = __builtin_amdgcn_update_dpp(x, x, 0xB1, 0xf, 0xf, false); break;
+    case 2: o = __builtin_amdgcn_update_dpp(x, x, 0x4E, 0xf, 0xf, false); break;
+    case 4: o = __builtin_amdgcn_ds_swizzle(x, (4 << 10) | 0x1f); break;
+    case 8: o = __builtin_amdgcn_ds_swizzle(x, (8 << 10) | 0x1f); break;
+    case 16: o = __builtin_amdgcn_ds_swizzle(x, (16 << 10) | 0x1f); break;
+    default: o = __shfl_xor(x, 32, WAVE); break;
+  }
+  return __builtin_bit_cast(float, o);
+}
+template <int R>
+__device__ __forceinline__ void bitonic_regs(float (&v)[R], int lane, int P) {
+#pragma unroll
+  for (int k = 2; k <= 64 * R; k <<= 1) {
+    if (k > P) continue;
+#pragma unroll
+    for (int j = k >> 1; j > 0; j >>= 1) {
+      if (j < 64) {
+        const bool lower = (lane & j) == 0;
+#pragma unroll
+        for (int r = 0; r < R; ++r) {
+          const float o = lane_xor(v[r], j);
+          const float a = lower ? v[r] : o, b = lower ? o : v[r];
+          const bool up = ((64 * r + lane) & k) == 0;
+          v[r] = ((a > b) == up) ? o : v[r];
+        }
+      } else {
+#pragma unroll
+        for (int r = 0; r < R; ++r) {
+          if (r & (j >> 6)) continue;
+          const int q = r | (j >> 6);
+          const float a = v[r], b = v[q];
+          const bool up = ((64 * r) & k) == 0;
+          if ((a > b) == up) { v[r] = b; v[q] = a; }
+        }
+      }
+    }
+  }
+}
+
+template <int CH, int R>
 __global__ void __launch_bounds__(256) importance_kernel(const float* __restrict__ z, const float* __restrict__ w,
                                                          const float* __restrict__ u, int64_t B, int n, int N,
                                                          int P, float eps, float* __restrict__ z_new,
@@ -43,8 +88,10 @@
                                                          int64_t* __restrict__ inds_out) {
   extern __shared__ __attribute__((aligned(16))) float smem[];
   const int lane = threadIdx.x & 63, wv = threadIdx.x >> 6;
-  const int per_wave = (n + 1) * 2 + ((n + P + 3) & ~3);
-  float* s_cdf = smem + wv * per_wave;
+  const int row = R ? ((n + N + 3) & ~3) : 0;
+  const int per_wave = row + (((n + 1) * 2 + ((n + P + 3) & ~3) + 3) & ~3);
+  float* s_row = smem + wv * per_wave;
+  float* s_cdf = s_row + row;
   float* s_zmid = s_cdf + (n + 1);
   float* s_all = s_zmid + (n + 1);
   for (int64_t ray = blockIdx.x * 4 + wv; ray < B; ray += (int64_t)gridDim.x * 4) {
@@ -88,7 +135,9 @@
     __builtin_amdgcn_wave_barrier();
     if (cdf_out) for (int i = lane; i <= n; i += WAVE) cdf_out[ray * (n + 1) + i] = s_cdf[i];
     bool new_nan = false;
-    for (int j = lane; j < N; j += WAVE) {
+    float vn[R ? R : 1];
+    (void)vn;
+    auto sample = [&](int j) -> float {
       const float uj = u[ray * N + j];
       const bool unan = uj != uj;
       int lo = 0, hi = n + 1;
@@ -108,6 +157,13 @@
       if (z_new) z_new[ray * N + j] = zn;
       if (inds_out) inds_out[ray * N + j] = inds;
       s_all[n + j] = zn;
+      return zn;
+    };
+    if constexpr (R == 0) {
+      for (int j = lane; j < N; j += WAVE) sample(j);
+    } else {
+#pragma unroll
+      for (int r = 0; r < R; ++r) vn[r] = (64 * r + lane < N) ? sample(64 * r + lane) : __builtin_inff();
     }
     __builtin_amdgcn_s_waitcnt(0);
     __builtin_amdgcn_wave_barrier();
@@ -116,7 +172,39 @@
       float* s_new = s_all + n;
       bool asc = !new_nan;
       for (int i = lane; i + 1 < n; i += WAVE) asc = asc && (s_all[i] <= s_all[i + 1]);
-      if (__all(asc)) {
+      if (R > 0 && __all(asc)) {
+        if constexpr (R > 0) {
+          bitonic_regs<R>(vn, lane, P);
+#pragma unroll
+          for (int r = 0; r < R; ++r)
+            if (64 * r + lane < N) s_new[64 * r + lane] = vn[r];
+          __builtin_amdgcn_s_waitcnt(0);
+          __builtin_amdgcn_wave_barrier();
+          for (int i = lane; i < n; i += WAVE) {
+            const float v = s_all[i];
+            int lo = 0, hi = N;
+            while (lo < hi) { const int mid = (lo + hi) >> 1; if (s_new[mid] < v) lo = mid + 1; else hi = mid; }
+            s_row[i + lo] = v;
+          }
+#pragma unroll
+          for (int r = 0; r < R; ++r) {
+            const int j = 64 * r + lane;
+            if (j < N) {
+              int lo = 0, hi = n;
+              while (lo < hi) { const int mid = (lo + hi) >> 1; if (s_all[mid] <= vn[r]) lo = mid + 1; else hi = mid; }
+              s_row[j + lo] = vn[r];
+            }
+          }
+          __builtin_amdgcn_s_waitcnt(0);
+          __builtin_amdgcn_wave_barrier();
+          float* out = z_merged + ray * tot;
+          if ((tot & 3) == 0 && (reinterpret_cast<uintptr_t>(z_merged) & 15) == 0) {
+            for (int i = lane; 4 * i < tot; i += WAVE) reinterpret_cast<float4*>(out)[i] = reinterpret_cast<const float4*>(s_row)[i];
+          } else {
+            for (int i = lane; i < tot; i += WAVE) out[i] = s_row[i];
+          }
+        }
+      } else if (__all(asc)) {
         for (int i = N + lane; i < P; i += WAVE) s_new[i] = __builtin_inff();
         __builtin_amdgcn_s_waitcnt(0);
         __builtin_amdgcn_wave_barrier();
@@ -199,11 +287,15 @@
   NERF_REQUIRE(z && weights && u, NERF_E_NULL, "nerf_importance_sample: z/weights/u is NULL");
   int P = 2;
   while (P < N) P <<= 1;
-  const int per_wave = (n + 1) * 2 + ((n + P + 3) & ~3);
+  const int R = (g_importance_variant && z_merged) ? (P < 64 ? 1 : P / 64) : 0;
+  const int row = R ? ((n + N + 3) & ~3) : 0;
+  const int per_wave = row + (((n + 1) * 2 + ((n + P + 3) & ~3) + 3) & ~3);
   const int lds = per_wave * 4 * (int)sizeof(float);
   return with_int_up_to<1, 2, 3, 4>((n + 63) / 64, [&](auto ch) {
-    return launch<importance_kernel<decltype(ch)::value>>("nerf_importance_sample", dim3(wave_per_ray_grid(B, 256 * 8)), dim3(256),
-                                                          lds, as_stream(stream), z, weights, u, B, n, N, P, eps, z_new, z_merged,
-                                                          cdf, inds);
+    return with_int_up_to<0, 1, 2, 4, 8>(R, [&](auto r) {
+      return launch<importance_kernel<decltype(ch)::value, decltype(r)::value>>("nerf_importance_sample", dim3(wave_per_ray_grid(B, 256 * 8)),
+                                                                                dim3(256), lds, as_stream(stream), z, weights, u, B, n, N, P,
+                                                                                eps, z_new, z_merged, cdf, inds);
+    });
   });
 }
diff --git a/nerf_meets_mlx_amd/models/NeRF.py b/nerf_meets_mlx_amd/models/NeRF.py
--- a/nerf_meets_mlx_amd/models/NeRF.py
+++ b/nerf_meets_mlx_amd/models/NeRF.py
@@ -55,6 +55,10 @@
         self._packed = None
         self._dirty = True
         self._packed_version = -1
+        self._param_gen = 0
+        self._fold = None
+        self._fold_gen = None
+        self.fold_fills = 0
         self._ws: Dict[str, torch.Tensor] = {}
         self.name: Optional[str] = None
         self._gen = 0
@@ -89,9 +93,11 @@
         with torch.no_grad():
             self.params.copy_(flat.to(self.device, torch.float32).reshape(-1))
         self._dirty = True
+        self._param_gen += 1
 
     def mark_updated(self):
         self._dirty = True
+        self._param_gen += 1
 
     def activation_generation(self) -> int:
         return self._acts_gen
@@ -119,6 +125,19 @@
         finally:
             lib.nerf_set_option(b"train_fold", before)
 
+    def _folded_product(self) -> Optional[torch.Tensor]:
+        lib = N.lib()
+        if not self._can_fold or lib.nerf_get_option(b"fold_once") != 1:
+            return None
+        gen = (self._param_gen, self.params._version)
+        if self._fold is None:
+            self._fold = torch.empty(N.FOLD_FLOATS, dtype=torch.float32, device=self.device)
+        if gen != self._fold_gen:
+            N.check(lib.nerf_mlp_fold(C.byref(self.arch), N.ptr(self.params), N.ptr(self._fold), N.stream()))
+            self._fold_gen = gen
+            self.fold_fills += 1
+        return self._fold
+
     def packed(self) -> torch.Tensor:
         lib = N.lib()
         if self._packed is None:
@@ -130,8 +149,12 @@
             self._packed = torch.empty(nbytes, dtype=torch.uint8, device=self.device)
         form = self.train_form()
         if self._dirty or self.params._version != self._packed_version or form != self._packed_form:
+            fold = self._folded_product()
             with self._form(form):
-                N.check(lib.nerf_mlp_pack(C.byref(self.arch), N.ptr(self.params), N.ptr(self._packed), N.stream()))
+                if fold is None:
+                    N.check(lib.nerf_mlp_pack(C.byref(self.arch), N.ptr(self.params), N.ptr(self._packed), N.stream()))
+                else:
+                    N.check(lib.nerf_mlp_pack_fold(C.byref(self.arch), N.ptr(self.params), N.ptr(fold), N.ptr(self._packed), N.stream()))
             self._dirty = False
             self._packed_version = self.params._version
             self._packed_form = form
```

New measurement: 1.406 million, median of 3. No clear change (+0.7%).
